# calebki/phylostan

Hardware: AMD Instinct MI355X
Metric: log-lik+grad evals/sec (HKY+W4, 69 taxa) at 1/2/4/8 MI355X; HBM-BW fraction (higher is better)
Workload: dtype f64; 1 GPU; fluA HKY+W4 strict clock, 8192 parameter draws per step; taxa=69, patterns=238, patterns_per_rank=238, categories=4, branches=136, parallelism=replicas1

## Files before the change

### include/phylo_hip_diag.h

```cpp
#ifndef PHYLO_HIP_DIAG_H
#define PHYLO_HIP_DIAG_H

#include "phylo_hip.h"

#ifdef __cplusplus
extern "C" {
#endif

int phy_program_info(const phy_ctx* ctx, int* nsteps, int* nslots, int* depth, int* nblocks);

int phy_plan_records(int S, const int32_t* peel, int rooted, int C, int R, int cols, int cap, int recompute,
                     int32_t* program, int32_t* records, int* nmat, int* n_chunks);

int phy_set_clade_compression(phy_ctx* ctx, int mode);
int phy_clade_compression(const phy_ctx* ctx, int* mode, int* facts, int* clades);

int phy_clade_plan(int S, int P, int C, int rooted, const uint8_t* tipcodes, const int32_t* peel, int R, int cap,
                   int recompute, int mode, int* facts, int* clades, int32_t* program, int32_t* records,
                   int32_t* mat_branch, int32_t* cls_of, int32_t* members, int32_t* rep);

#define PHY_PLAN_QUAD 13
#define PHY_PLAN_CLADE 17
#define PHY_PLAN_LAUNCH 29
#define PHY_PLAN_FACTS 36
int phy_plan_sweep(int S, int P, int C, int rooted, const uint8_t* tipcodes, const int32_t* peel, int max_draws,
                   int cu_count, int wg_budget, int cols, int lds_budget, int deep, int recompute, int clade_mode,
                   int rescaling, int n_draws, int* facts);

int phy_timing_start(phy_ctx* ctx);
int phy_timing_read(phy_ctx* ctx, double* total_ms, int* launches);

int phy_set_tuning(phy_ctx* ctx, int wg_budget, int cols, int lds_budget);

int phy_lds_plan(const phy_ctx* ctx, int* n_chunks, int* matrices_per_chunk, int* lds_bytes);

int phy_columns_per_lane(const phy_ctx* ctx);

int phy_set_deep_stack(phy_ctx* ctx, int mode);
int phy_deep_stack_in_lds(const phy_ctx* ctx);

int phy_set_recompute(phy_ctx* ctx, int on);
int phy_recomputed_partials(const phy_ctx* ctx);

int phy_set_engine(phy_ctx* ctx, int mode);
int phy_engine(const phy_ctx* ctx);

int phy_set_rescaling(phy_ctx* ctx, int on);
int phy_rescaling(const phy_ctx* ctx);

int phy_class_info(const phy_ctx* ctx, long long* classes, int* levels, int* root_classes, long long* stage,
                   long long* staged, int* tiles, int* spans);

int phy_class_clades(const phy_ctx* ctx, int* fused_levels, int* clades, long long* largest);

int phy_class_chain(const phy_ctx* ctx, int* levels, int* lowest, int* top_classes);

int phy_class_fused(const phy_ctx* ctx, int* level_pairs, int* chunk_spans, int* parent_order_levels);

int phy_quad_plan(const phy_ctx* ctx, int* waves, int* span, int* slots);

int phy_geo_info(const phy_geo_ctx* ctx, int* levels, int* widest_level, int* lds_bytes, int* threads,
                 int* workgroups);
int phy_geo_sweeps(phy_geo_ctx* ctx, int n_draws, int* sweeps);
int phy_geo_trees_info(const phy_geo_trees_ctx* ctx, int* widest_level, int* max_levels, int* groups, int* threads,
                       int* lds_bytes, int* workgroups);
int phy_forest_info(const phy_forest_ctx* ctx, int* cols, int* cap_m, int* max_chunks, int* min_chunks,
                    int* max_depth, int* min_depth, int* deep_in_lds, int* lds_bytes);
int phy_forest_plan(int S, int P, int C, int rooted, int model, const uint8_t* tipcodes, const double* weights, int T,
                    const int32_t* peels, int max_rows, int cu_count, int* facts, int* chunks, int* depths);

#ifdef __cplusplus
}
#endif
#endif
```

### phylostan_amd/_lib.py

```python
import ctypes
import importlib.abc
import importlib.machinery
import importlib.util
import os

_HERE = os.path.dirname(os.path.abspath(__file__))
LIB_PATH = os.environ.get("PHYLO_HIP_LIB") or os.path.join(_HERE, "libphylo_hip.so")

PHY_JC69, PHY_HKY, PHY_GTR = 0, 1, 2

_lib = None

_c_double_p = ctypes.POINTER(ctypes.c_double)
_c_int_p = ctypes.POINTER(ctypes.c_int)

SIGNATURES = {
    "phy_create": (ctypes.c_int, [ctypes.c_int, ctypes.c_int, ctypes.c_int, ctypes.c_int, ctypes.c_int,
                                  ctypes.c_void_p, ctypes.c_void_p, ctypes.c_void_p, ctypes.c_int,
                                  ctypes.c_int, ctypes.POINTER(ctypes.c_void_p)]),
    "phy_create_multi": (ctypes.c_int, [ctypes.c_int, ctypes.c_int, ctypes.c_int, ctypes.c_int, ctypes.c_int,
                                        ctypes.c_void_p, ctypes.c_void_p, ctypes.c_void_p, ctypes.c_int,
                                        ctypes.c_int, ctypes.c_void_p, ctypes.POINTER(ctypes.c_void_p)]),
    "phy_destroy": (ctypes.c_int, [ctypes.c_void_p]),
    "phy_last_error": (ctypes.c_char_p, []),
    "phy_num_branches": (ctypes.c_int, [ctypes.c_void_p]),
    "phy_output_len": (ctypes.c_int, [ctypes.c_void_p]),
    "phy_program_info": (ctypes.c_int, [ctypes.c_void_p, _c_int_p, _c_int_p, _c_int_p, _c_int_p]),
    "phy_plan_records": (ctypes.c_int, [ctypes.c_int, ctypes.c_void_p, ctypes.c_int, ctypes.c_int, ctypes.c_int,
                                        ctypes.c_int, ctypes.c_int, ctypes.c_int, ctypes.c_void_p,
                                        ctypes.c_void_p, _c_int_p, _c_int_p]),
    "phy_clade_plan": (ctypes.c_int, [ctypes.c_int] * 4 + [ctypes.c_void_p, ctypes.c_void_p] + [ctypes.c_int] * 4 +
                       [ctypes.c_void_p] * 8),
    "phy_plan_sweep": (ctypes.c_int, [ctypes.c_int] * 4 + [ctypes.c_void_p, ctypes.c_void_p] + [ctypes.c_int] * 10 +
                       [ctypes.c_void_p]),
    "phy_set_clade_compression": (ctypes.c_int, [ctypes.c_void_p, ctypes.c_int]),
    "phy_clade_compression": (ctypes.c_int, [ctypes.c_void_p, _c_int_p, ctypes.c_void_p, ctypes.c_void_p]),
    "phy_eval": (ctypes.c_int, [ctypes.c_void_p, ctypes.c_int, ctypes.c_void_p, ctypes.c_void_p,
                                ctypes.c_void_p, ctypes.c_void_p]),
    "phy_eval_submit": (ctypes.c_int, [ctypes.c_void_p, ctypes.c_int, ctypes.c_void_p, ctypes.c_void_p]),
    "phy_eval_wait": (ctypes.c_int, [ctypes.c_void_p, ctypes.c_void_p]),
    "phy_eval_device": (ctypes.c_int, [ctypes.c_void_p, ctypes.c_int, ctypes.c_void_p, ctypes.c_void_p,
                                       ctypes.c_void_p, ctypes.c_void_p, ctypes.c_void_p]),
    "phy_pruning_loglik": (ctypes.c_double, [ctypes.c_void_p, ctypes.c_void_p, ctypes.c_void_p,
                                             ctypes.c_void_p]),
    "phy_sync": (ctypes.c_int, [ctypes.c_void_p]),
    "phy_timing_start": (ctypes.c_int, [ctypes.c_void_p]),
    "phy_timing_read": (ctypes.c_int, [ctypes.c_void_p, _c_double_p, _c_int_p]),
    "phy_set_tuning": (ctypes.c_int, [ctypes.c_void_p, ctypes.c_int, ctypes.c_int, ctypes.c_int]),
    "phy_lds_plan": (ctypes.c_int, [ctypes.c_void_p, _c_int_p, _c_int_p, _c_int_p]),
    "phy_columns_per_lane": (ctypes.c_int, [ctypes.c_void_p]),
    "phy_set_deep_stack": (ctypes.c_int, [ctypes.c_void_p, ctypes.c_int]),
    "phy_deep_stack_in_lds": (ctypes.c_int, [ctypes.c_void_p]),
    "phy_set_recompute": (ctypes.c_int, [ctypes.c_void_p, ctypes.c_int]),
    "phy_recomputed_partials": (ctypes.c_int, [ctypes.c_void_p]),
    "phy_set_engine": (ctypes.c_int, [ctypes.c_void_p, ctypes.c_int]),
    "phy_set_output": (ctypes.c_int, [ctypes.c_void_p, ctypes.c_int]),
    "phy_engine": (ctypes.c_int, [ctypes.c_void_p]),
    "phy_set_rescaling": (ctypes.c_int, [ctypes.c_void_p, ctypes.c_int]),
    "phy_rescaling": (ctypes.c_int, [ctypes.c_void_p]),
    "phy_class_info": (ctypes.c_int, [ctypes.c_void_p, ctypes.POINTER(ctypes.c_longlong), _c_int_p, _c_int_p,
                                      ctypes.POINTER(ctypes.c_longlong), ctypes.POINTER(ctypes.c_longlong),
                                      _c_int_p, _c_int_p]),
    "phy_class_clades": (ctypes.c_int, [ctypes.c_void_p, _c_int_p, _c_int_p, ctypes.POINTER(ctypes.c_longlong)]),
    "phy_class_chain": (ctypes.c_int, [ctypes.c_void_p, _c_int_p, _c_int_p, _c_int_p]),
    "phy_quad_plan": (ctypes.c_int, [ctypes.c_void_p, _c_int_p, _c_int_p, _c_int_p]),
    "phy_class_fused": (ctypes.c_int, [ctypes.c_void_p, _c_int_p, _c_int_p, _c_int_p]),
    "phy_geo_info": (ctypes.c_int, [ctypes.c_void_p, _c_int_p, _c_int_p, _c_int_p, _c_int_p, _c_int_p]),
    "phy_geo_sweeps": (ctypes.c_int, [ctypes.c_void_p, ctypes.c_int, ctypes.c_void_p]),
    "phy_geo_trees_info": (ctypes.c_int, [ctypes.c_void_p] + [_c_int_p] * 6),
    "phy_forest_info": (ctypes.c_int, [ctypes.c_void_p] + [_c_int_p] * 8),
    "phy_forest_plan": (ctypes.c_int, [ctypes.c_int] * 5 + [ctypes.c_void_p, ctypes.c_void_p, ctypes.c_int,
                                                           ctypes.c_void_p, ctypes.c_int, ctypes.c_int] +
                        [ctypes.c_void_p] * 3),
}


GEO_SIGNATURES = {
    "phy_geo_create": (ctypes.c_int, [ctypes.c_int, ctypes.c_int, ctypes.c_void_p, ctypes.c_void_p, ctypes.c_int,
                                      ctypes.c_int, ctypes.POINTER(ctypes.c_void_p)]),
    "phy_geo_destroy": (ctypes.c_int, [ctypes.c_void_p]),
    "phy_geo_num_branches": (ctypes.c_int, [ctypes.c_void_p]),
    "phy_geo_output_len": (ctypes.c_int, [ctypes.c_void_p]),
    "phy_geo_eval": (ctypes.c_int, [ctypes.c_void_p, ctypes.c_int, ctypes.c_void_p, ctypes.c_void_p,
                                    ctypes.c_void_p]),
    "phy_geo_summary_len": (ctypes.c_int, [ctypes.c_void_p]),
    "phy_geo_eval_summaries": (ctypes.c_int, [ctypes.c_void_p, ctypes.c_int, ctypes.c_void_p, ctypes.c_void_p,
                                              ctypes.c_void_p, ctypes.c_void_p]),
    "phy_geo_trees_create": (ctypes.c_int, [ctypes.c_int, ctypes.c_int, ctypes.c_void_p, ctypes.c_int, ctypes.c_void_p,
                                            ctypes.c_void_p, ctypes.c_void_p, ctypes.c_int, ctypes.c_int,
                                            ctypes.POINTER(ctypes.c_void_p)]),
    "phy_geo_trees_destroy": (ctypes.c_int, [ctypes.c_void_p]),
    "phy_geo_trees_num_trees": (ctypes.c_int, [ctypes.c_void_p]),
    "phy_geo_trees_output_len": (ctypes.c_int, [ctypes.c_void_p]),
    "phy_geo_trees_summary_len": (ctypes.c_int, [ctypes.c_void_p]),
    "phy_geo_trees_eval": (ctypes.c_int, [ctypes.c_void_p, ctypes.c_int, ctypes.c_void_p, ctypes.c_void_p,
                                          ctypes.c_void_p]),
    "phy_geo_trees_eval_summaries": (ctypes.c_int, [ctypes.c_void_p, ctypes.c_int, ctypes.c_void_p, ctypes.c_void_p,
                                                    ctypes.c_void_p, ctypes.c_void_p]),
    "phy_geo_trees_clock_output_len": (ctypes.c_int, [ctypes.c_void_p]),
    "phy_geo_trees_eval_clock": (ctypes.c_int, [ctypes.c_void_p, ctypes.c_int, ctypes.c_void_p, ctypes.c_void_p,
                                                ctypes.c_void_p, ctypes.c_void_p]),
    "phy_geo_trees_eval_clock_summaries": (ctypes.c_int, [ctypes.c_void_p, ctypes.c_int, ctypes.c_void_p,
                                                          ctypes.c_void_p, ctypes.c_void_p, ctypes.c_void_p,
                                                          ctypes.c_void_p]),
}


FOREST_SIGNATURES = {
    "phy_forest_create": (ctypes.c_int, [ctypes.c_int] * 5 + [ctypes.c_void_p, ctypes.c_void_p, ctypes.c_int,
                                                             ctypes.c_void_p, ctypes.c_int, ctypes.c_int,
                                                             ctypes.POINTER(ctypes.c_void_p)]),
    "phy_forest_destroy": (ctypes.c_int, [ctypes.c_void_p]),
    "phy_forest_num_trees": (ctypes.c_int, [ctypes.c_void_p]),
    "phy_forest_num_branches": (ctypes.c_int, [ctypes.c_void_p]),
    "phy_forest_output_len": (ctypes.c_int, [ctypes.c_void_p]),
# ... 76 lines not shown
```

### phylostan_amd/csrc/phylo_hip.hip

```cpp

#include <hip/hip_runtime.h>

#include <cmath>
#include <cstdio>
#include <cstring>
#include <memory>
#include <type_traits>

#include "sweep_plan.h"
#include "forest_plan.h"
#include "geo_plan.h"

namespace {

#ifndef PHY_EPI_U
#define PHY_EPI_U 4
#endif
struct Step {
  int x, y;
  int mxo, myo, mvo;
  int gx, gy, gv;
  int vso;
  uint32_t xso, yso;
  int fl, xd, vd, m0, mn, rd;
// ... 79 lines not shown

template <int CTRL>
__device__ __forceinline__ double dpp_d(double v) {
  const int lo = __builtin_amdgcn_mov_dpp(__double2loint(v), CTRL, 0xF, 0xF, false);
  const int hi = __builtin_amdgcn_mov_dpp(__double2hiint(v), CTRL, 0xF, 0xF, false);
  return __hiloint2double(hi, lo);
}
__device__ __forceinline__ void swap32(double& a, double& b) {
  auto l = __builtin_amdgcn_permlane32_swap(__double2loint(a), __double2loint(b), false, false);
  auto h = __builtin_amdgcn_permlane32_swap(__double2hiint(a), __double2hiint(b), false, false);
  a = __hiloint2double(h[0], l[0]);
  b = __hiloint2double(h[1], l[1]);
}
__device__ __forceinline__ void swap16(double& a, double& b) {
  auto l = __builtin_amdgcn_permlane16_swap(__double2loint(a), __double2loint(b), false, false);
  auto h = __builtin_amdgcn_permlane16_swap(__double2hiint(a), __double2hiint(b), false, false);
  a = __hiloint2double(h[0], l[0]);
  b = __hiloint2double(h[1], l[1]);
}
constexpr int DPP_ROW_ROR8 = 0x128;
constexpr int DPP_ROW_HALF_MIRROR = 0x141;
constexpr int DPP_QUAD_XOR1 = 0xB1;
constexpr int DPP_QUAD_XOR2 = 0x4E;

__device__ __forceinline__ double reduce16(double (&v)[16], int lane) {
#pragma unroll
  for (int k = 0; k < 8; ++k) {
    swap32(v[k], v[k + 8]);
    v[k] += v[k + 8];
  }
#pragma unroll
  for (int k = 0; k < 4; ++k) {
    swap16(v[k], v[k + 4]);
    v[k] += v[k + 4];
  }
  {
    const bool hi = lane & 8;
#pragma unroll
    for (int k = 0; k < 2; ++k) {
      const double send = hi ? v[k] : v[k + 2];
      const double keep = hi ? v[k + 2] : v[k];
      v[k] = keep + dpp_d<DPP_ROW_ROR8>(send);
    }
  }
  {
    const bool hi = lane & 4;
    const double send = hi ? v[0] : v[1];
    const double keep = hi ? v[1] : v[0];
    v[0] = keep + dpp_d<DPP_ROW_HALF_MIRROR>(send);
  }
  double s = v[0];
  s += dpp_d<DPP_QUAD_XOR1>(s);
  s += dpp_d<DPP_QUAD_XOR2>(s);
  return s;
}

__device__ __forceinline__ int reduce16_entry(int lane) {
  return ((lane >> 5) & 1) * 8 + ((lane >> 4) & 1) * 4 + ((lane >> 3) & 1) * 2 + ((lane >> 2) & 1);
}

struct SweepArgs {
  const uint8_t* tips;
  const double* weights;
  const double* pmat;
  const double* model;
  double2* scratch;
  double2* dstk;
  double* gslot;
  double* sslot;
  double* site_ll;
  double* out;
  const int* mat_branch;
  const double* eig;
  double* inner;
  int S, P, Ppad, C, nsteps, nslots, ndeep, ndl, nblk, nmat, R, cap_m;
  int B, outlen, g_direct;
  unsigned long long extra;
  int fin;
  const double* blens;
  double* grows;
  long long grows_stride;
  int qfused, kind;
  int* escr;
  union {
    const int* cc;
    const int* tree_of_row;
  };
  union {
    int cc_ncl;
    int fo_stride;
  };
  int cc_nL, cc_ncol, cc_spos, cc_pre, cc_cnt;
};

__device__ __forceinline__ __amdgpu_buffer_rsrc_t make_rsrc(const void* base, uint32_t bytes) {
  const uint64_t a = reinterpret_cast<uint64_t>(base);
  const uint32_t lo = __builtin_amdgcn_readfirstlane((uint32_t)a);
  const uint32_t hi = __builtin_amdgcn_readfirstlane((uint32_t)(a >> 32));
  const uint32_t n = __builtin_amdgcn_readfirstlane(bytes);
  void* p = reinterpret_cast<void*>(((uint64_t)hi << 32) | lo);
  return __builtin_amdgcn_make_buffer_rsrc(p, (short)0, (int)n, 0x00020000);
}
constexpr int LOAD_NT = 2;
#ifndef PHY_STORE_AUX
#define PHY_STORE_AUX 0
#endif
constexpr int STORE_AUX = PHY_STORE_AUX;
__device__ __forceinline__ V4 ld_v4(__amdgpu_buffer_rsrc_t srd, uint32_t off, uint32_t half) {
  const auto lo = __builtin_amdgcn_raw_buffer_load_b128(srd, off, 0, LOAD_NT);
  const auto hi = __builtin_amdgcn_raw_buffer_load_b128(srd, off, half, LOAD_NT);
  V4 r;
  r.x = __hiloint2double((int)lo[1], (int)lo[0]);
  r.y = __hiloint2double((int)lo[3], (int)lo[2]);
  r.z = __hiloint2double((int)hi[1], (int)hi[0]);
  r.w = __hiloint2double((int)hi[3], (int)hi[2]);
  return r;
}

__device__ __forceinline__ void st_v4(__amdgpu_buffer_rsrc_t srd, uint32_t off, uint32_t half, const V4& v) {
  typedef unsigned u4 __attribute__((ext_vector_type(4)));
  const u4 lo = {(unsigned)__double2loint(v.x), (unsigned)__double2hiint(v.x), (unsigned)__double2loint(v.y),
                 (unsigned)__double2hiint(v.y)};
  const u4 hi = {(unsigned)__double2loint(v.z), (unsigned)__double2hiint(v.z), (unsigned)__double2loint(v.w),
                 (unsigned)__double2hiint(v.w)};
  __builtin_amdgcn_raw_buffer_store_b128(lo, srd, off, 0, STORE_AUX);
  __builtin_amdgcn_raw_buffer_store_b128(hi, srd, off, half, STORE_AUX);
}

__device__ __forceinline__ int v4_exp(const V4& v) {
  const double m = fmax(fmax(v.x, v.y), fmax(v.z, v.w));
  return m > 0.0 ? __builtin_amdgcn_frexp_exp(m) - 1 : 0;
}
__device__ __forceinline__ V4 vldexp(const V4& a, int n) {
  return {ldexp(a.x, n), ldexp(a.y, n), ldexp(a.z, n), ldexp(a.w, n)};
}
__device__ __forceinline__ int ld_exp(__amdgpu_buffer_rsrc_t srd, uint32_t off) {
  return (int)__builtin_amdgcn_raw_buffer_load_b32(srd, off, 0, LOAD_NT);
}
__device__ __forceinline__ void st_exp(__amdgpu_buffer_rsrc_t srd, uint32_t off, int e) {
  __builtin_amdgcn_raw_buffer_store_b32((unsigned)e, srd, off, 0, STORE_AUX);
}

#define WAIT_VMCNT0() __builtin_amdgcn_s_waitcnt(0x0F70)

template <int K>
__device__ __forceinline__ void pvec_k(const double* __restrict__ M, const V4 (&v)[K], V4 (&r)[K]) {
  const double2 a01 = *reinterpret_cast<const double2*>(M + 0), a23 = *reinterpret_cast<const double2*>(M + 2);
  const double2 b01 = *reinterpret_cast<const double2*>(M + 4), b23 = *reinterpret_cast<const double2*>(M + 6);
  const double2 c01 = *reinterpret_cast<const double2*>(M + 8), c23 = *reinterpret_cast<const double2*>(M + 10);
  const double2 d01 = *reinterpret_cast<const double2*>(M + 12), d23 = *reinterpret_cast<const double2*>(M + 14);
#pragma unroll
  for (int k = 0; k < K; ++k) {
    const V4 x = v[k];
    r[k].x = fma(d01.x, x.w, fma(c01.x, x.z, fma(b01.x, x.y, a01.x * x.x)));
    r[k].y = fma(d01.y, x.w, fma(c01.y, x.z, fma(b01.y, x.y, a01.y * x.x)));
    r[k].z = fma(d23.x, x.w, fma(c23.x, x.z, fma(b23.x, x.y, a23.x * x.x)));
    r[k].w = fma(d23.y, x.w, fma(c23.y, x.z, fma(b23.y, x.y, a23.y * x.x)));
  }
}
template <int K>
__device__ __forceinline__ void ptvec_k(const double* __restrict__ M, const V4 (&v)[K], V4 (&r)[K]) {
  const double2 a01 = *reinterpret_cast<const double2*>(M + 0), a23 = *reinterpret_cast<const double2*>(M + 2);
  const double2 b01 = *reinterpret_cast<const double2*>(M + 4), b23 = *reinterpret_cast<const double2*>(M + 6);
  const double2 c01 = *reinterpret_cast<const double2*>(M + 8), c23 = *reinterpret_cast<const double2*>(M + 10);
  const double2 d01 = *reinterpret_cast<const double2*>(M + 12), d23 = *reinterpret_cast<const double2*>(M + 14);
#pragma unroll
  for (int k = 0; k < K; ++k) {
    const V4 x = v[k];
    r[k].x = fma(a23.y, x.w, fma(a23.x, x.z, fma(a01.y, x.y, a01.x * x.x)));
    r[k].y = fma(b23.y, x.w, fma(b23.x, x.z, fma(b01.y, x.y, b01.x * x.x)));
    r[k].z = fma(c23.y, x.w, fma(c23.x, x.z, fma(c01.y, x.y, c01.x * x.x)));
    r[k].w = fma(d23.y, x.w, fma(d23.x, x.z, fma(d01.y, x.y, d01.x * x.x)));
  }
}

// ... 196 lines not shown
        E[2] = dpp_d<0xAA>(Ek);
        E[3] = dpp_d<0xFF>(Ek);
        double T[4];
#pragma unroll
        for (int j = 0; j < 4; ++j) {
          const double g0 = dpp_d<0x00>(g[j]), g1 = dpp_d<0x55>(g[j]), gg2 = dpp_d<0xAA>(g[j]),
                       g3 = dpp_d<0xFF>(g[j]);
          T[j] = fma(sV[12 + k], g3, fma(sV[8 + k], gg2, fma(sV[4 + k], g1, fma(sV[k], g0, 0.0))));
        }
#pragma unroll
        for (int l = 0; l < 4; ++l) {
          double hh = 0.0;
#pragma unroll
          for (int j = 0; j < 4; ++j) hh = fma(T[j], sVi[l * 4 + j], hh);
          const double ri = srinv[k * 4 + l];
          const double phi = ri == 0.0 ? t * Ek : (Ek - E[l]) * ri;
          m[l] = fma(hh, phi, m[l]);
        }
      }
    }
    if (near_any) {
      const RowsG rows{a.grows + (size_t)draw * a.grows_stride};
      double m2[4] = {0.0, 0.0, 0.0, 0.0};
      for (int idx = vt >> 2; idx < C * B; idx += QG_THREADS / 4) {
        const int c = idx / B, b = idx - c * B;
        const double t = mdl[10 + c] * bl[b], Ek = exp(slam[k] * t);
        double g[4];
        rows(idx, k, g);
        double T[4];
#pragma unroll
        for (int j = 0; j < 4; ++j) {
          const double g0 = dpp_d<0x00>(g[j]), g1 = dpp_d<0x55>(g[j]), gg2 = dpp_d<0xAA>(g[j]),
                       g3 = dpp_d<0xFF>(g[j]);
          T[j] = fma(sV[12 + k], g3, fma(sV[8 + k], gg2, fma(sV[4 + k], g1, fma(sV[k], g0, 0.0))));
        }
        const double E[4] = {dpp_d<0x00>(Ek), dpp_d<0x55>(Ek), dpp_d<0xAA>(Ek), dpp_d<0xFF>(Ek)};
#pragma unroll
        for (int l = 0; l < 4; ++l) {
          if (!phi_is_near(slam[k], slam[l])) continue;
          double hh = 0.0;
#pragma unroll
          for (int j = 0; j < 4; ++j) hh = fma(T[j], sVi[l * 4 + j], hh);
          const double d = slam[k] - slam[l];
          m2[l] = fma(hh, phi_near(d, t, Ek, E[l]) - (Ek - E[l]) * srinv[k * 4 + l], m2[l]);
        }
      }
#pragma unroll
      for (int l = 0; l < 4; ++l) m[l] += m2[l];
    }
#pragma unroll
    for (int u = 0; u < 2; ++u) {
      swap32(m[u], m[u + 2]);
      m[u] += m[u + 2];
    }
    swap16(m[0], m[1]);
    m[0] += m[1];
    m[0] += dpp_d<DPP_ROW_ROR8>(m[0]);
    m[0] += dpp_d<0x124>(m[0]);
    if ((lane & 12) == 0) part[vw * 16 + k * 4 + ((lane >> 5) & 1) * 2 + ((lane >> 4) & 1)] = m[0];
  }
  __syncthreads();
  if (tid < 16) {
    double acc = part[tid];
    for (int w = 1; w < QG_THREADS / 64; ++w) acc += part[w * 16 + tid];
    sM[tid] = acc;
  }
  __syncthreads();
  if (tid < 16) sW[tid] = w_entry(sM, sV, sVi, tid);
  __syncthreads();
  if (tid != 0) return;
  double W[16];
  for (int kk = 0; kk < 16; ++kk) W[kk] = sW[kk];
  q_tail(W, e + EIG_Q, e[EIG_S], mdl, out + o, out + o);
}

#ifdef PHY_STEPTIME
#ifndef TT_DRAW0
#define TT_DRAW0 0
#endif
constexpr int TT_DRAWS = 64, TT_EV = 1024;
__device__ unsigned long long g_tt[TT_DRAWS * 16][TT_EV];
#define TT_MARK(i)                                                                   \
  do {                                                                               \
    if (draw >= TT_DRAW0 && draw < TT_DRAW0 + TT_DRAWS && lane == 0)                 \
      g_tt[(draw - TT_DRAW0) * 16 + wv][(i)] = __builtin_amdgcn_s_memtime();         \
  } while (0)
#else
#define TT_MARK(i) do {} while (0)
#endif
template <int MAXT, int K, bool DL, bool RS, bool CC = false, bool FO = false>
__global__ void __launch_bounds__(MAXT) __attribute__((amdgpu_waves_per_eu(MAXT <= 512 ? PHY_WPE2 : 4)))
    sweep_kernel(SweepArgs a, const int* __restrict__ prog) {
  static_assert(!CC || (K == 2 && !RS), "compressed clades: the two-column unscaled sweep only");
  static_assert(!FO || (!CC && !RS), "forest: the unscaled sweep without clades only");
  const int* matbr = a.mat_branch;
  if constexpr (FO) {
    const int t = __builtin_amdgcn_readfirstlane(a.tree_of_row[blockIdx.y]);
    prog += (size_t)t * a.fo_stride;
    matbr += (size_t)t * a.nmat;
  }
  extern __shared__ __attribute__((aligned(16))) unsigned char lds_raw[];
  const int lane = threadIdx.x & (WAVE - 1);
  const int C = a.C, nsteps = a.nsteps, nmat = a.nmat;
  const int wv = __builtin_amdgcn_readfirstlane(threadIdx.x >> 6);
  const int c = wv;
  const int nthreads = blockDim.x;
  const int draw = blockIdx.y;
  const int wg = blockIdx.y * gridDim.x + blockIdx.x;
  const int rec = a.R * 4;
  const int ncolwg = C * WAVE;

  unsigned char* tipl = lds_raw;
  double* tvec = reinterpret_cast<double*>(lds_raw + tip_nib_bytes(a.S, K));
  double* mats0 = tvec + 64;
  if (threadIdx.x < 64) {
    const unsigned b = threadIdx.x >> 2, j = threadIdx.x & 3;
    const unsigned m = b < 4 ? (1u << b) : (unsigned)(a.extra >> (4 * (b - 4))) & 15u;
    tvec[threadIdx.x] = (double)((m >> j) & 1u);
  }
  double* mats = mats0 + (size_t)c * a.cap_m * rec;
  const int ndl = DL ? a.ndeep : a.ndl;
  double* tail0 = mats0 + (size_t)C * a.cap_m * rec;
  const size_t tstride = tail_doubles(K, ndl);

  const double* mdl = a.model + (size_t)draw * (10 + 2 * C);
  const V4 pi = {mdl[0], mdl[1], mdl[2], mdl[3]};
  const double ps_c = mdl[10 + C + c];
  const double* pmat_c = a.pmat + ((size_t)draw * C + c) * nmat * rec;
  const size_t entry2 = (size_t)K * 2 * ncolwg;
  double2* scr = a.scratch + (size_t)wg * a.nslots * entry2;
  double2* dsk = a.dstk + (size_t)wg * a.ndeep * entry2;
  const uint32_t scr_bytes = (uint32_t)((size_t)a.nslots * entry2 * 16);
  const uint32_t dsk_bytes = (uint32_t)((size_t)a.ndeep * entry2 * 16);
  const __amdgpu_buffer_rsrc_t srd_scr = make_rsrc(scr, scr_bytes);
  const __amdgpu_buffer_rsrc_t srd_dsk = make_rsrc(dsk, dsk_bytes);
  const int colw = c * WAVE + lane;
  const uint32_t half_bytes = (uint32_t)ncolwg * 16u;
  const uint32_t estr = (uint32_t)(K * 2 * ncolwg * 16);
  uint32_t lcol[K];
#pragma unroll
  for (int k = 0; k < K; ++k) lcol[k] = (uint32_t)((k * 2 * ncolwg + colw) * 16);
  auto ent = [&](bool use, int e) __attribute__((always_inline)) -> uint32_t {
    return use ? (uint32_t)e * estr : OOB;
  };
  uint32_t lofs[K];
  __amdgpu_buffer_rsrc_t srd_esc = srd_scr;
  uint32_t eofs[K];
  int Eacc[K];
  if constexpr (RS) {
    int* esc = a.escr + (size_t)wg * a.nslots * K * ncolwg;
    srd_esc = make_rsrc(esc, (uint32_t)((size_t)a.nslots * K * ncolwg * 4));
  }
  auto put =[&](double2* base, int e, int k, const V4& v) __attribute__((always_inline)) {
    double2* d = base + ((size_t)e * K + k) * 2 * ncolwg + colw;
    d[0] = make_double2(v.x, v.y);
    d[ncolwg] = make_double2(v.z, v.w);
  };
  double2* dlw = reinterpret_cast<double2*>(tail0 + (size_t)wv * tstride);
  auto dput = [&](int e, int k, const V4& v) __attribute__((always_inline)) {
    double2* d = dlw + (size_t)(e * K + k) * 2 * WAVE + lane;
    d[0] = make_double2(v.x, v.y);
    d[WAVE] = make_double2(v.z, v.w);
  };
  auto dget = [&](int e, int k) __attribute__((always_inline)) -> V4 {
    const double2* d = dlw + (size_t)(e * K + k) * 2 * WAVE + lane;
    const double2 lo = d[0], hi = d[WAVE];
    return V4(lo.x, lo.y, hi.x, hi.y);
  };

  double* gs = a.gslot + ((size_t)wg * C + c) * nmat * 16;
  const int e = reduce16_entry(lane);
  const bool gowner = (lane & 3) == 0;
  char* const gsl = reinterpret_cast<char*>(gs + e);
  bool gstore = gowner, gadd = false;
  auto step_at = [&](int s) __attribute__((always_inline)) -> Step { return ld_step<K>(prog, s, rec * 8, estr); };

  double acc_ll = 0.0, acc_dps = 0.0;
  V4 acc_f = {0.0, 0.0, 0.0, 0.0};

  int cur = -1;
  auto ensure_chunk = [&](const Step& st) {
    const int lo = st.m0, n = st.mn;
    if (lo == cur) return;
    const double2* src = reinterpret_cast<const double2*>(pmat_c + (size_t)lo * rec);
    double2* dst = reinterpret_cast<double2*>(mats);
    const int q2 = n * rec / 2;
    for (int k0 = lane; k0 < q2; k0 += WAVE * 8) {
      double2 buf[8];
#pragma unroll
      for (int u = 0; u < 8; ++u) {
        const int k = k0 + u * WAVE;
        buf[u] = (k < q2) ? src[k] : make_double2(0.0, 0.0);
      }
#pragma unroll
      for (int u = 0; u < 8; ++u) {
        const int k = k0 + u * WAVE;
        if (k < q2) dst[k] = buf[u];
      }
    }
    WAIT_VMCNT0();
    cur = lo;
  };
  const unsigned char* const matb = reinterpret_cast<const unsigned char*>(mats);
  auto mrec = [&](int mo) __attribute__((always_inline)) -> const double* {
    return reinterpret_cast<const double*>(matb + mo);
  };
  const unsigned char* const tipw = tipl + (lane >> 1);
  const unsigned nsh = (lane & 1) * 4;
  auto tipb = [&](int to, int k) __attribute__((always_inline)) -> unsigned {
    return __builtin_amdgcn_ubfe((unsigned)tipw[to + k * (WAVE / 2)], nsh, 4u);
  };
  auto look = [&](int mo, unsigned b) __attribute__((always_inline)) -> V4 {
    const unsigned char* p = matb + mo + (b << 5);
    const double2 lo = *reinterpret_cast<const double2*>(p);
    const double2 hi = *reinterpret_cast<const double2*>(p + 16);
    return {lo.x, lo.y, hi.x, hi.y};
  };
  auto gacc = [&](int go, const V4 (&r)[K], const V4 (&p)[K]) __attribute__((always_inline)) {
    double v[16];
    v[0] = r[0].x * p[0].x;  v[1] = r[0].x * p[0].y;  v[2] = r[0].x * p[0].z;  v[3] = r[0].x * p[0].w;
    v[4] = r[0].y * p[0].x;  v[5] = r[0].y * p[0].y;  v[6] = r[0].y * p[0].z;  v[7] = r[0].y * p[0].w;
    v[8] = r[0].z * p[0].x;  v[9] = r[0].z * p[0].y;  v[10] = r[0].z * p[0].z; v[11] = r[0].z * p[0].w;
    v[12] = r[0].w * p[0].x; v[13] = r[0].w * p[0].y; v[14] = r[0].w * p[0].z; v[15] = r[0].w * p[0].w;
#pragma unroll
    for (int k = 1; k < K; ++k) {
      v[0] = fma(r[k].x, p[k].x, v[0]);   v[1] = fma(r[k].x, p[k].y, v[1]);
      v[2] = fma(r[k].x, p[k].z, v[2]);   v[3] = fma(r[k].x, p[k].w, v[3]);
      v[4] = fma(r[k].y, p[k].x, v[4]);   v[5] = fma(r[k].y, p[k].y, v[5]);
      v[6] = fma(r[k].y, p[k].z, v[6]);   v[7] = fma(r[k].y, p[k].w, v[7]);
      v[8] = fma(r[k].z, p[k].x, v[8]);   v[9] = fma(r[k].z, p[k].y, v[9]);
      v[10] = fma(r[k].z, p[k].z, v[10]); v[11] = fma(r[k].z, p[k].w, v[11]);
      v[12] = fma(r[k].w, p[k].x, v[12]); v[13] = fma(r[k].w, p[k].y, v[13]);
      v[14] = fma(r[k].w, p[k].z, v[14]); v[15] = fma(r[k].w, p[k].w, v[15]);
    }
    const double sum = reduce16(v, lane);
    double* const d = reinterpret_cast<double*>(gsl + (uint32_t)go);
    if (gstore) *d = sum;
    if (gadd) unsafeAtomicAdd(d, sum);
  };

  const int VG = gridDim.x, vg = blockIdx.x;
  const int trips = CC ? a.nblk + 2 : (a.nblk - vg + VG - 1) / VG;
  const uint32_t cw = (uint32_t)c * (WAVE * 16);
  const uint32_t plane_half = (uint32_t)a.nblk * (estr / 2);
  const uint32_t cwp = (uint32_t)c * (uint32_t)a.nblk * (WAVE * K * 16);
  for (int trip = 0; trip < trips; ++trip) {
    const bool passLF = CC && trip == 0, passLR = CC && trip == trips - 1;
    const int blk = CC ? ((passLF || passLR) ? a.nblk : trip - 1) : vg + trip * VG;
    const int f0 = CC ? ((passLF || passLR) ? 0 : a.cc_nL) : 0;
    const int f1 = CC ? (passLF ? a.cc_nL : passLR ? 0 : nsteps) : nsteps;
    const int plim = (CC && (passLF || passLR)) ? a.nblk * (WAVE * K) + a.cc_ncol : a.P;
    TT_MARK(trip * 320 + 0);
#pragma unroll
    for (int k = 0; k < K; ++k) lofs[k] = (blk * WAVE * K + k * WAVE + lane < plim) ? lcol[k] : OOB;
    if constexpr (RS) {
#pragma unroll
      for (int k = 0; k < K; ++k) {
        eofs[k] = (blk * WAVE * K + k * WAVE + lane < a.P) ? (uint32_t)((k * ncolwg + colw) * 4) : OOB;
        Eacc[k] = 0;
      }
    }
    __syncthreads();
    {
      const uint32_t* src = reinterpret_cast<const uint32_t*>(a.tips);
      uint32_t* dst = reinterpret_cast<uint32_t*>(tipl);
      const int rowq = a.Ppad / 8;
      constexpr int wq = WAVE * K / 8;
      const int nq = a.S * wq;
      const int nthr = C * WAVE, t0 = c * WAVE + lane;
      for (int k0 = t0; k0 < nq; k0 += nthr * 8) {
        uint32_t buf[8];
#pragma unroll
        for (int u = 0; u < 8; ++u) {
          const int k = k0 + u * nthr;
          buf[u] = (k < nq) ? src[(size_t)(k / wq) * rowq + blk * wq + (k % wq)] : 0u;
        }
#pragma unroll
        for (int u = 0; u < 8; ++u) {
          const int k = k0 + u * nthr;
          if (k < nq) dst[k] = buf[u];
        }
      }
    }
    __syncthreads();
    WAIT_VMCNT0();
    TT_MARK(trip * 320 + 1);

    V4 top[K], proot[K];
#pragma unroll
    for (int k = 0; k < K; ++k) top[k] = proot[k] = {0.0, 0.0, 0.0, 0.0};
    #define GATHER(ch, so, out) do {                                                         \
      const int* gt_ = a.cc + CC_HDR + ((-2 - (ch)) * a.nblk + blk) * (WAVE * K) + lane;     \
      uint32_t gc_[K];                                                                       \
      _Pragma("unroll")                                                                      \
      for (int k = 0; k < K; ++k) gc_[k] = (uint32_t)gt_[k * WAVE] + cw;                     \
      _Pragma("unroll")                                                                      \
      for (int k = 0; k < K; ++k) out[k] = ld_v4(srd_scr, gc_[k] + (so), half_bytes);        \
      WAIT_VMCNT0();                                                                         \
    } while (0)
    #define FSTEP(s, dcur, dnext, st, sn) do {                                            \
      {                                                                                   \
        const bool more = s + 1 < f1;                                                     \
        sn = step_at(more ? s + 1 : s);                     \
          \
        const bool need = more && (sn.fl & F_XDEEP) && sn.xd >= ndl;                      \
        if (!DL)                                                                                                      \
      _Pragma("unroll")                                                                                               \
        for (int k = 0; k < K; ++k) dnext[k] = ld_v4(srd_scr, lofs[k] + (need ? sn.xso : OOB), half_bytes);    \
      }                                                                                                               \
      ensure_chunk(st);                                                                                               \
      const int x = st.x, y = st.y, fl = st.fl, vso = st.vso;                      \
      V4 ax[K], ay[K], pv[K];                                                                                         \
      if (y >= 0) {                                                                                                   \
        const int my = st.myo;                                                                                    \
      _Pragma("unroll")                                                                                               \
        for (int k = 0; k < K; ++k) ay[k] = look(my, tipb(y, k));                                                     \
      } else if (CC && y < -1) {                                                                                      \
        GATHER(y, st.yso, ay);                                                                                        \
      } else {                                                                                                        \
      _Pragma("unroll")                                                                                               \
        for (int k = 0; k < K; ++k) ay[k] = top[k];                                                                   \
      }                                                                                                               \
      if (x >= 0) {                                                                                                   \
        const int mx = st.mxo;                                                                                    \
      _Pragma("unroll")                                                                                               \
        for (int k = 0; k < K; ++k) ax[k] = look(mx, tipb(x, k));                                                     \
      } else if (CC && x < -1) {                                                                                      \
        GATHER(x, st.xso, ax);                                                                                        \
      } else if (CC ? y != -1 : y >= 0) {                                                                             \
      _Pragma("unroll")                                                                                               \
        for (int k = 0; k < K; ++k) ax[k] = top[k];                                                                   \
      } else {                                                                                                        \
        {                                                                                                             \
          const int xd = st.xd;                                                                                \
          if (DL || xd < ndl) {                                                                                       \
      _Pragma("unroll")                                                                                               \
            for (int k = 0; k < K; ++k) ax[k] = dget(xd, k);                                                          \
          } else {                                                                                                    \
      _Pragma("unroll")                                                                                               \
            for (int k = 0; k < K; ++k) ax[k] = dcur[k];                                                              \
          }                                                                                                           \
        }                                                                                                             \
      }                                                                                                               \
      _Pragma("unroll")                                                                                               \
      for (int k = 0; k < K; ++k) pv[k] = vmul(ax[k], ay[k]);                                                         \
      if (vso >= 0) {                                                                                                 \
        V4 av[K];                                                                                                     \
        if (fl & F_MV) {                                                                                              \
          pvec_k<K>(mrec(st.mvo), pv, av);                                                                        \
        } else {                                                 \
      _Pragma("unroll")                                                                                               \
          for (int k = 0; k < K; ++k) av[k] = pv[k];                                                                  \
        }                                                                                                             \
        if constexpr (RS) {                           \
          if (!(fl & F_NOSTORE)) {                                                                                    \
      _Pragma("unroll")                                                                                               \
            for (int k = 0; k < K; ++k) {                                                                             \
              const int ev = v4_exp(av[k]);                                                                           \
              av[k] = vldexp(av[k], -ev);                                                                             \
              Eacc[k] += ev;                                                                                          \
              st_exp(srd_esc, eofs[k] + ((uint32_t)vso >> 3), ev);                                                    \
            }                                                                                                         \
          }                                                                                                           \
        }                                                                                                             \
      _Pragma("unroll")                                                                                               \
        for (int k = 0; k < K; ++k) if (!(fl & F_NOSTORE)) st_v4(srd_scr, lofs[k] + (uint32_t)vso, half_bytes, av[k]);                                    \
        if (fl & F_VDEEP) {                                                                                           \
          const int dp = st.vd;                                                                                \
          if (DL || dp < ndl)                                          \
          for (int k = 0; k < K; ++k) dput(dp, k, av[k]);                                                             \
        }                                                                                                             \
      _Pragma("unroll")                                                                                               \
        for (int k = 0; k < K; ++k) top[k] = av[k];                                                                   \
      } else {                                                                                                        \
      _Pragma("unroll")                                                                                               \
        for (int k = 0; k < K; ++k) proot[k] = pv[k];                                                                 \
      }                                                                                                               \
    } while (0)
    {
      V4 dA[K], dB[K];
#pragma unroll
// ... 12 lines not shown
    TT_MARK(trip * 320 + 152);

    double fp[K];
    int Est[K], Ed[K];
    if constexpr (RS) {
#pragma unroll
      for (int k = 0; k < K; ++k) {
        fp[k] = vdot(pi, proot[k]);
        *reinterpret_cast<int*>(&tail0[(size_t)wv * tstride + k * WAVE + lane]) = fp[k] > 0.0 ? Eacc[k] : INT_MIN;
      }
      __syncthreads();
#pragma unroll
      for (int k = 0; k < K; ++k) {
        int es = INT_MIN;
        for (int cc = 0; cc < C; ++cc)
          es = max(es, *reinterpret_cast<const int*>(&tail0[(size_t)cc * tstride + k * WAVE + lane]));
        Est[k] = es == INT_MIN ? 0 : es;
      }
      __syncthreads();
#pragma unroll
      for (int k = 0; k < K; ++k) {
        Ed[k] = min(Eacc[k] - Est[k], RS_DMAX);
        fp[k] = ldexp(fp[k], Ed[k]);
        tail0[(size_t)wv * tstride + k * WAVE + lane] = ps_c * fp[k];
      }
    } else {
#pragma unroll
    for (int k = 0; k < K; ++k) {
      fp[k] = vdot(pi, proot[k]);
      tail0[(size_t)wv * tstride + k * WAVE + lane] = ps_c * fp[k];
    }
    }
    __syncthreads();
    double L[K];
#pragma unroll
    for (int k = 0; k < K; ++k) {
      L[k] = 0.0;
      for (int cc = 0; cc < C; ++cc) L[k] += tail0[(size_t)cc * tstride + k * WAVE + lane];
    }
    __syncthreads();
    TT_MARK(trip * 320 + 153);
    V4 topr[K];
#pragma unroll
    for (int k = 0; k < K; ++k) {
      const int i = blk * WAVE * K + k * WAVE + lane;
      const bool live = i < a.P;
      const double wt = a.weights[i];
      double lnL = live ? log(L[k]) : 0.0;
      if constexpr (RS) {
        if (live) lnL = fma((double)Est[k], 0.69314718055994530942, lnL);
      }
      if (c == 0) {
        acc_ll += wt * lnL;
        if (a.site_ll != nullptr && live) a.site_ll[(size_t)draw * a.P + i] = lnL;
      }
      const double sc = live ? wt / L[k] : 0.0;
      double s_c = sc * ps_c;
      if constexpr (RS) s_c = ldexp(s_c, Ed[k]);
      acc_dps = fma(sc, fp[k], acc_dps);
      acc_f.x = fma(s_c, proot[k].x, acc_f.x);
      acc_f.y = fma(s_c, proot[k].y, acc_f.y);
      acc_f.z = fma(s_c, proot[k].z, acc_f.z);
      acc_f.w = fma(s_c, proot[k].w, acc_f.w);
      topr[k] = vscale(pi, s_c);
    }

    struct CSet {
      V4 lx[K], ly[K], lr[K];
      Step st;
      int ex[K], ey[K];
    };
    #define LOAD_SET(s, r) do {                                                  \
      const bool ok = s >= rlo;                                                  \
      r.st = step_at(ok ? s : rlo);                                              \
                                                      \
      const uint32_t xso = ok ? r.st.xso : OOB, yso = ok ? r.st.yso : OOB;       \
      const bool lr = ok && (r.st.fl & F_VDEEP) && r.st.vd >= ndl;               \
      const int vd = r.st.vd;                                                    \
      uint32_t cx_[K], cy_[K];                                                   \
      _Pragma("unroll")                                                          \
      for (int k = 0; k < K; ++k) cx_[k] = cy_[k] = lofs[k];                     \
      if constexpr (CC) {   \
        if (ok && r.st.x < -1) {                                                 \
          const int* gt_ = a.cc + CC_HDR + ((-2 - r.st.x) * a.nblk + blk) * (WAVE * K) + lane;  \
      _Pragma("unroll")                                                          \
          for (int k = 0; k < K; ++k) cx_[k] = (uint32_t)gt_[k * WAVE] + cw;     \
          WAIT_VMCNT0();                                                         \
        }                                                                        \
        if (ok && r.st.y < -1) {                                                 \
          const int* gt_ = a.cc + CC_HDR + ((-2 - r.st.y) * a.nblk + blk) * (WAVE * K) + lane;  \
      _Pragma("unroll")                                                          \
          for (int k = 0; k < K; ++k) cy_[k] = (uint32_t)gt_[k * WAVE] + cw;     \
          WAIT_VMCNT0();                                                         \
        }                                                                        \
      }                                                                          \
      _Pragma("unroll")                                                          \
      for (int k = 0; k < K; ++k) {                                              \
        r.lx[k] = ld_v4(srd_scr, cx_[k] + xso, half_bytes);                      \
        r.ly[k] = ld_v4(srd_scr, cy_[k] + yso, half_bytes);                      \
        if constexpr (!DL)                                                       \
          r.lr[k] = ld_v4(srd_dsk, lcol[k] + ent(lr, vd), half_bytes);            \
        if constexpr (RS) {                                                      \
          r.ex[k] = ld_exp(srd_esc, eofs[k] + (xso >> 3));                       \
          r.ey[k] = ld_exp(srd_esc, eofs[k] + (yso >> 3));                       \
        }                                                                        \
      }                                                                          \
    } while (0)
    #define REBUILD(cst, out) do {   \
      V4 p_[K];                                                                                     \
      _Pragma("unroll")                                                                             \
      for (int k = 0; k < K; ++k)                                                                   \
        p_[k] = vmul(look(cst.mxo, tipb(cst.x, k)), look(cst.myo, tipb(cst.y, k)));                   \
      pvec_k<K>(mrec(cst.mvo), p_, out);                                                            \
    } while (0)
    #define CHAIN_UP(vst, in, out) do {                                                   \
      V4 pu_[K];                                                                          \
      if (vst.x >= 0) {                                                                   \
      _Pragma("unroll")                                                                   \
        for (int k = 0; k < K; ++k) pu_[k] = vmul(look(vst.mxo, tipb(vst.x, k)), in[k]);  \
      } else {                                                                            \
      _Pragma("unroll")                                                                   \
        for (int k = 0; k < K; ++k) pu_[k] = vmul(in[k], look(vst.myo, tipb(vst.y, k))); \
      }                                                                                   \
      pvec_k<K>(mrec(vst.mvo), pu_, out);                                                 \
    } while (0)
    #define REBUILDN(vst, s, d, out) do {                                                 \
      if (d == 1) {                                                                       \
        REBUILD(vst, out);                                                                \
      } else {                                                                            \
        const Step cb_ = step_at(s - d);                                                          \
        V4 acc_[K];                                                                       \
        REBUILD(cb_, acc_);                                                               \
        for (int j_ = d - 1; j_ >= 2; --j_) {                                             \
          const Step v_ = step_at(s - j_);                                                        \
          CHAIN_UP(v_, acc_, acc_);                                                       \
        }                                                                                 \
        CHAIN_UP(vst, acc_, out);                                                         \
      }                                                                                   \
    } while (0)
    #define PLANE_PUT(ch, po, r) do {                                                    \
      const int* sp_ = a.cc + a.cc_spos + ((-2 - (ch)) * a.nblk + blk) * (WAVE * K) + lane;  \
      uint32_t so_[K];                                                                   \
      _Pragma("unroll")                                                                  \
      for (int k = 0; k < K; ++k) so_[k] = (uint32_t)sp_[k * WAVE] + cwp + (uint32_t)(po);  \
      WAIT_VMCNT0();                                                                     \
      _Pragma("unroll")                                                                  \
      for (int k = 0; k < K; ++k) st_v4(srd_scr, so_[k], plane_half, r[k]);              \
    } while (0)
    #define RSTEP_V(s, cs, cn, XT, YT) do {                                               \
      const Step& st = cs.st;                                                     \
      ensure_chunk(st);                                                           \
      const int fl = st.fl;                                                       \
      V4 rv[K], ax[K], ay[K], q[K], rx[K], ry[K];                                 \
      unsigned bx[K], by[K];                                                      \
      if (fl & F_VDEEP) {                                                         \
        const int vd = st.vd;                                                     \
        if (DL || vd < ndl) {                                                     \
      _Pragma("unroll")                                                           \
          for (int k = 0; k < K; ++k) rv[k] = dget(vd, k);                        \
        } else {                                                                  \
      _Pragma("unroll")                                                           \
          for (int k = 0; k < K; ++k) rv[k] = cs.lr[k];                           \
        }                                                                         \
      } else {                                                                    \
      _Pragma("unroll")                                                           \
        for (int k = 0; k < K; ++k) rv[k] = topr[k];                              \
      }                                                                           \
      if (XT) {                                                                   \
        const int mx = st.mxo, x = st.x;                                          \
      _Pragma("unroll")                                                           \
        for (int k = 0; k < K; ++k) {                                             \
          bx[k] = tipb(x, k);                                                     \
          ax[k] = look(mx, bx[k]);                                                \
        }                                                                         \
      } else if (YT && (fl & F_PREVREC)) {   \
        REBUILDN(cn.st, s, st.rd, ax);                                                 \
      } else {                                                                         \
      _Pragma("unroll")                                                                \
        for (int k = 0; k < K; ++k) ax[k] = cs.lx[k];                                  \
      }                                                                           \
      if (YT) {                                                                   \
        const int my = st.myo, y = st.y;                                          \
      _Pragma("unroll")                                                           \
        for (int k = 0; k < K; ++k) {                                             \
          by[k] = tipb(y, k);                                                     \
          ay[k] = look(my, by[k]);                                                \
        }                                                                         \
      } else if (fl & F_PREVREC) {   \
        REBUILDN(cn.st, s, st.rd, ay);                                         \
      } else {                                                                 \
      _Pragma("unroll")                                                        \
        for (int k = 0; k < K; ++k) ay[k] = cs.ly[k];                          \
      }                                                                           \
      if (fl & F_MV) {                                                            \
        V4 pv[K];                                                                 \
      _Pragma("unroll")                                                           \
        for (int k = 0; k < K; ++k) pv[k] = vmul(ax[k], ay[k]);                   \
        ptvec_k<K>(mrec(st.mvo), rv, q);                                          \
        gacc(st.gv, rv, pv);                          \
      } else {                     \
      _Pragma("unroll")                                                           \
        for (int k = 0; k < K; ++k) q[k] = rv[k];                                 \
      }                                                                           \
      _Pragma("unroll")                                                           \
      for (int k = 0; k < K; ++k) {                                               \
        rx[k] = vmul(q[k], ay[k]);                                                \
        ry[k] = vmul(q[k], ax[k]);                                                \
        if constexpr (RS) {     \
          if (!XT) rx[k] = vldexp(rx[k], -cs.ex[k]);                              \
          if (!YT) ry[k] = vldexp(ry[k], -cs.ey[k]);                              \
        }                                                                         \
      }                                                                           \
      if (XT) {                                                                   \
        V4 tv[K];                                                                 \
      _Pragma("unroll")                                                           \
        for (int k = 0; k < K; ++k) tv[k] = tipvec_l(tvec, bx[k]);                \
        gacc(st.gx, rx, tv);                                                      \
      }                                                                           \
      if (YT) {                                                                   \
        V4 tv[K];                                                                 \
      _Pragma("unroll")                                                           \
        for (int k = 0; k < K; ++k) tv[k] = tipvec_l(tvec, by[k]);                \
        gacc(st.gy, ry, tv);                                                      \
      }                                                                           \
                                  \
      if (CC && !XT && st.x < -1) PLANE_PUT(st.x, st.gx, rx);                     \
      if (CC && !YT && st.y < -1) PLANE_PUT(st.y, st.gy, ry);                     \
      if (!XT && !YT) {   \
        if (CC && (st.x < -1 || st.y < -1)) {   \
          if (st.y == -1) {                                                       \
      _Pragma("unroll")                                                           \
            for (int k = 0; k < K; ++k) topr[k] = ry[k];                          \
          } else {                                                                \
      _Pragma("unroll")                                                           \
            for (int k = 0; k < K; ++k) topr[k] = rx[k];                          \
          }                                                                       \
        } else {                                                                  \
        const int dp = st.xd;                                                     \
      _Pragma("unroll")                                                           \
        for (int k = 0; k < K; ++k) {                                             \
          if (DL || dp < ndl) dput(dp, k, rx[k]); else put(dsk, dp, k, rx[k]);    \
          topr[k] = ry[k];                                                        \
        }                                                                         \
        }                                                                         \
      } else if (!YT) {                                                           \
      _Pragma("unroll")                                                           \
        for (int k = 0; k < K; ++k) topr[k] = ry[k];                              \
      } else if (!XT) {                                                           \
      _Pragma("unroll")                                                           \
        for (int k = 0; k < K; ++k) topr[k] = rx[k];                              \
      }                                                                           \
    } while (0)
    #define RSTEP(s, cs, cn) do {                        \
      const int xt_ = cs.st.x >= 0, yt_ = cs.st.y >= 0;  \
      if (xt_ && yt_) RSTEP_V(s, cs, cn, true, true);    \
      else if (xt_) RSTEP_V(s, cs, cn, true, false);     \
      else if (yt_) RSTEP_V(s, cs, cn, false, true);     \
      else RSTEP_V(s, cs, cn, false, false);             \
    } while (0)
    const int nseg = CC ? (passLF ? 0 : passLR ? a.cc_ncl : 1) : 1;
    for (int sg = nseg - 1; sg >= 0; --sg) {
      int rlo = CC ? a.cc_nL : 0, rhi = nsteps - 1;
      if constexpr (CC) {
        if (passLR) {
          rlo = a.cc[4 * sg];
          rhi = a.cc[4 * sg + 1];
          const int mm = a.cc[4 * sg + 3];
          uint32_t pre[K], cnt[K];
#pragma unroll
          for (int k = 0; k < K; ++k) {
            pre[k] = (uint32_t)a.cc[a.cc_pre + sg * (WAVE * K) + k * WAVE + lane] + cwp +
                     (uint32_t)(nsteps + sg * a.nblk) * estr;
            cnt[k] = (uint32_t)a.cc[a.cc_cnt + sg * (WAVE * K) + k * WAVE + lane];
          }
#pragma unroll
          for (int k = 0; k < K; ++k) topr[k] = {0.0, 0.0, 0.0, 0.0};
          for (int t = 0; t < mm; t += CC_ROUNDS_U) {
            V4 rr[CC_ROUNDS_U][K];
#pragma unroll
            for (int u = 0; u < CC_ROUNDS_U; ++u)
#pragma unroll
              for (int k = 0; k < K; ++k)
                rr[u][k] = ld_v4(srd_scr, (uint32_t)(t + u) < cnt[k] ? pre[k] + (uint32_t)(t + u) * 16u : OOB, plane_half);
#pragma unroll
            for (int u = 0; u < CC_ROUNDS_U; ++u)
#pragma unroll
              for (int k = 0; k < K; ++k) {
                topr[k].x += rr[u][k].x;
                topr[k].y += rr[u][k].y;
                topr[k].z += rr[u][k].z;
                topr[k].w += rr[u][k].w;
              }
          }
          WAIT_VMCNT0();
        }
      }
      int s = rhi;
      CSet A, Bs;
      LOAD_SET(s, A);
      for (;;) {
        TT_MARK(trip * 320 + 154 + (nsteps - 1 - s));
        LOAD_SET(s - 1, Bs);
        RSTEP(s, A, Bs);
        if (--s < rlo) break;
        TT_MARK(trip * 320 + 154 + (nsteps - 1 - s));
        LOAD_SET(s - 1, A);
        RSTEP(s, Bs, A);
        if (--s < rlo) break;
      }
    }
    WAIT_VMCNT0();
    TT_MARK(trip * 320 + 310);
    if constexpr (CC) {
      gstore = gowner && (trip == 0 || trip == trips - 2);
      gadd = gowner && !gstore;
    } else {
    gstore = false;
    gadd = gowner;
    }
  }

  acc_ll = wave_sum(acc_ll);
  acc_dps = wave_sum(acc_dps);
  acc_f.x = wave_sum(acc_f.x);
  acc_f.y = wave_sum(acc_f.y);
  acc_f.z = wave_sum(acc_f.z);
  acc_f.w = wave_sum(acc_f.w);
  if (lane == 0) {
    double* ss = a.sslot + ((size_t)wg * C + c) * 8;
    ss[0] = acc_ll;
    ss[1] = acc_dps;
    ss[2] = acc_f.x;
    ss[3] = acc_f.y;
    ss[4] = acc_f.z;
    ss[5] = acc_f.w;
  }
  if (a.g_direct) {
    WAIT_VMCNT0();
    TT_MARK(990);
    double* innerL = mats0;
    double* scalL = mats0 + (size_t)C * a.B;
    if (a.fin) __syncthreads();
    const double* Qd = a.eig + (size_t)draw * EIG_LEN + EIG_Q;
    double* gout = a.grows + (size_t)draw * a.grows_stride;
    double* inner_d = a.inner + (size_t)draw * C * a.B;
    const int e16 = lane & 15, j = e16 >> 2, kk = e16 & 3;
    const double q0 = Qd[j * 4 + 0], q1 = Qd[j * 4 + 1], q2 = Qd[j * 4 + 2], q3 = Qd[j * 4 + 3];
    const int tot = nmat * 16;
    constexpr int U = PHY_EPI_U;
    for (int k0 = lane; k0 < tot; k0 += WAVE * U) {
      double g[U], qp[U];
      int bb[U];
#pragma unroll
      for (int u = 0; u < U; ++u) {
        const int k = k0 + u * WAVE;
        const int kc = k < tot ? k : lane;
// ... 720 lines not shown
    for (int w = 1; w < QFIN_THREADS / 64; ++w) acc += wpart[w][t];
    __hip_atomic_store(hp + t, acc, __ATOMIC_RELAXED, __HIP_MEMORY_SCOPE_AGENT);
  }
  if (tid >= 128 && tid < 128 + C) {
    const int cc = tid - 128;
    double acc = 0.0;
    for (int j = 0; j < nb; ++j) acc = fma(blv[b0 + j], sinner[cc * bper + j], acc);
    __hip_atomic_store(hp + 16 + cc, acc, __ATOMIC_RELAXED, __HIP_MEMORY_SCOPE_AGENT);
  }
  if (sp == 0 && tid == 0) {
    const double ll = sred[0];
    out[0] = isfinite(ll) ? ll : -INFINITY;
    for (int cc = 0; cc < C; ++cc) out[1 + B + C + cc] = sred[cc * 8 + 1];
    for (int f = 0; f < 4; ++f) {
      double t = 0.0;
      for (int cc = 0; cc < C; ++cc) t += sred[cc * 8 + 2 + f];
      __hip_atomic_store(out + o + f, t, __ATOMIC_RELAXED, __HIP_MEMORY_SCOPE_AGENT);
    }
  }
  asm volatile("s_waitcnt vmcnt(0)" ::: "memory");
  __syncthreads();
  if (tid == 0) {
    const unsigned long long old = __hip_atomic_fetch_add(qa.cnt + draw, 1ull, __ATOMIC_RELAXED,
                                                          __HIP_MEMORY_SCOPE_AGENT);
    const bool last = ((old + 1) % (unsigned long long)nspl) == 0;
    handoff_acquire(last);
    s_last = last;
  }
  __syncthreads();
  if (!s_last) return;
  __builtin_amdgcn_fence(__ATOMIC_ACQUIRE, "wavefront");
  const double* pp = qa.part + (size_t)draw * nspl * (16 + C);
  auto ld1 = [](const double* q) { return __hip_atomic_load(q, __ATOMIC_RELAXED, __HIP_MEMORY_SCOPE_AGENT); };
  if (tid < 16) {
    double u[8];
    double acc = 0.0;
    for (int q0 = 0; q0 < nspl; q0 += 8) {
#pragma unroll
      for (int v = 0; v < 8; ++v) u[v] = q0 + v < nspl ? ld1(pp + (size_t)(q0 + v) * (16 + C) + tid) : 0.0;
#pragma unroll
      for (int v = 0; v < 8; ++v)
        if (q0 + v < nspl) acc = (q0 + v == 0) ? u[v] : acc + u[v];
    }
    sM[tid] = acc;
  }
  if (tid >= 64 && tid < 64 + C) {
    const int cc = tid - 64;
    double u[8];
    double acc = 0.0;
    for (int q0 = 0; q0 < nspl; q0 += 8) {
#pragma unroll
      for (int v = 0; v < 8; ++v) u[v] = q0 + v < nspl ? ld1(pp + (size_t)(q0 + v) * (16 + C) + 16 + cc) : 0.0;
#pragma unroll
      for (int v = 0; v < 8; ++v)
        if (q0 + v < nspl) acc = (q0 + v == 0) ? u[v] : acc + u[v];
    }
    out[1 + B + cc] = acc;
  }
  if (!qp) {
    if (tid < 10) out[o + 4 + tid] = 0.0;
    return;
  }
  __syncthreads();
  if (tid < 16) wpart[0][tid] = w_entry(sM, sV, sVi, tid);
  __syncthreads();
  if (tid != 0) return;
  double W[16];
  for (int t = 0; t < 16; ++t) W[t] = wpart[0][t];
  const double rt[4] = {ld1(out + o), ld1(out + o + 1), ld1(out + o + 2), ld1(out + o + 3)};
  q_tail(W, sQ, eg[EIG_S], mdl, rt, out + o);
}

}

namespace {
struct ClassEngine;
void free_class_engine(ClassEngine* e);
struct MultiState;
void free_multi(MultiState* m);

struct CladeBuffers {
  uint8_t* tips = nullptr;
  double* w = nullptr;
  int *prog = nullptr, *tab = nullptr;
  int *matbr = nullptr, *gpos = nullptr;
};
}

struct phy_ctx {
  Problem pb;
  Prefs prefs;
  SweepPlan plan;
  QuadPlan quad;
  CladePlan cc;
  CladeBuffers ccd;
  int device = 0;
  int wg_cap = 0;
  int *d_qprog = nullptr, *d_mprog = nullptr;
  double* d_qscr = nullptr;
  double* d_qfpart = nullptr;
  unsigned long long* d_qfcnt = nullptr;
  long qscr_wgs = 0;
  int* d_escr = nullptr;
  ClassEngine* ce = nullptr;
  MultiState* ms = nullptr;
  int compact = 0;
  double* d_grows = nullptr;
  hipStream_t stream = nullptr;
  hipEvent_t ev_nin = nullptr, ev_nout = nullptr;
  uint8_t* d_tips = nullptr;
  double* d_w = nullptr;
  int *d_prog = nullptr, *d_gpos = nullptr, *d_mat_branch = nullptr;
  double *d_pmat = nullptr, *d_eig = nullptr, *d_inner = nullptr;
  double *d_model = nullptr, *d_blens = nullptr, *d_out = nullptr, *d_site = nullptr;
  double* h_in = nullptr;
  double* h_out = nullptr;
  double* d_in = nullptr;
  int pending = 0;
  double2 *d_scratch = nullptr, *d_dstk = nullptr;
  double *d_gslot = nullptr, *d_sslot = nullptr;
  bool timing = false;
  std::vector<hipEvent_t> ev;
  int ev_used = 0, timed_n = 0;
  double timed_ms = 0.0;
};

namespace {

void free_ctx(phy_ctx* c) {
  if (!c) return;
  int dev_old = 0;
  (void)hipGetDevice(&dev_old);
  (void)hipSetDevice(c->device);
  void* ptrs[] = {c->d_tips,  c->d_w,     c->d_prog,    c->d_gpos,    c->d_mat_branch, c->d_pmat,
                  c->d_eig,   c->d_inner, c->d_model,   c->d_blens,   c->d_out,        c->d_site,
                  c->d_scratch, c->d_dstk, c->d_gslot,  c->d_sslot, c->d_grows, c->d_in, c->d_qprog, c->d_qscr,
                  c->d_qfpart, c->d_qfcnt, c->d_mprog, c->d_escr,
                  c->ccd.tips, c->ccd.w, c->ccd.prog, c->ccd.tab, c->ccd.matbr, c->ccd.gpos};
  for (void* p : ptrs)
    if (p) (void)hipFree(p);
  if (c->h_in) (void)hipHostFree(c->h_in);
  if (c->h_out) (void)hipHostFree(c->h_out);
  for (hipEvent_t e : c->ev) (void)hipEventDestroy(e);
  if (c->ev_nin) (void)hipEventDestroy(c->ev_nin);
  if (c->ev_nout) (void)hipEventDestroy(c->ev_nout);
  free_class_engine(c->ce);
  free_multi(c->ms);
  if (c->stream) (void)hipStreamDestroy(c->stream);
  (void)hipSetDevice(dev_old);
  delete c;
}

template <typename T>
int dalloc(T** p, size_t n) {
  if (n == 0) n = 1;
  hipError_t e = hipMalloc(reinterpret_cast<void**>(p), n * sizeof(T));
  if (e != hipSuccess)
    return fail(PHY_ENOMEM, std::string("hipMalloc ") + std::to_string(n * sizeof(T)) + " B: " +
                                hipGetErrorString(e));
  return PHY_OK;
}

template <typename T, typename U>
int upload(T* dst, const std::vector<U>& src) {
  static_assert(sizeof(T) == sizeof(U), "element sizes differ");
  HIP_TRY(hipMemcpy(dst, src.data(), src.size() * sizeof(U), hipMemcpyHostToDevice));
  return PHY_OK;
}

#include "class_engine.inc"

constexpr int PIN_DRAWS = 128;

struct SweepKernel { int K; bool lat, dl, rs, cc; const void* fn; };
const void* sweep_kernel_cc(bool dl);
const SweepKernel SWEEP_KERNELS[] = {
    {2, false, true, true, false, (const void*)sweep_kernel<512, 2, true, true>},
    {2, false, false, true, false, (const void*)sweep_kernel<512, 2, false, true>},
    {1, true, true, true, false, (const void*)sweep_kernel<512, 1, true, true>},
    {1, true, false, true, false, (const void*)sweep_kernel<512, 1, false, true>},
    {1, false, true, true, false, (const void*)sweep_kernel<1024, 1, true, true>},
    {1, false, false, true, false, (const void*)sweep_kernel<1024, 1, false, true>},
    {2, false, true, false, false, (const void*)sweep_kernel<512, 2, true, false>},
    {2, false, false, false, false, (const void*)sweep_kernel<512, 2, false, false>},
    {1, true, true, false, false, (const void*)sweep_kernel<512, 1, true, false>},
    {1, true, false, false, false, (const void*)sweep_kernel<512, 1, false, false>},
    {1, false, true, false, false, (const void*)sweep_kernel<1024, 1, true, false>},
    {1, false, false, false, false, (const void*)sweep_kernel<1024, 1, false, false>},
    {2, false, true, false, true, sweep_kernel_cc(true)},
    {2, false, false, false, true, sweep_kernel_cc(false)},
};
const void* sweep_kernel_for(int K, bool lat, bool dl, bool rs, bool cc) {
  for (const SweepKernel& k : SWEEP_KERNELS)
    if (k.K == K && k.lat == (lat && K == 1) && k.dl == dl && k.rs == rs && k.cc == cc) return k.fn;
  return nullptr;
}

int alloc_wg_buffers(phy_ctx* c, long cap);

int scratch_slots(const phy_ctx* c) {
  return c->cc.ncl > 0 ? std::max(c->pb.nslots, clade_nslots(c->cc, c->pb.S)) : c->pb.nslots;
}

int build_clade_plan(phy_ctx* c) {
  CladeBuffers& d = c->ccd;
  void* old[] = {d.tips, d.w, d.prog, d.tab, d.matbr, d.gpos};
  for (void* p : old)
    if (p) (void)hipFree(p);
  d = CladeBuffers();
  c->plan.cc_ok = false;
  const Problem& pb = c->pb;
  int rc = select_clades(pb, c->prefs.cc_mode, c->cc);
  if (rc) return rc;
  const CladePlan& cp = c->cc;
  if (cp.ncl == 0) return PHY_OK;
  const std::vector<uint8_t> tips = pack_tips(pb, &cp);
  std::vector<double> w(pb.Ppad + CC_COLS, 0.0);
  std::copy(pb.w.begin(), pb.w.end(), w.begin());
  std::vector<int> gpos(pb.B, -1);
  for (int m = 0; m < cp.nmat; ++m) gpos[cp.mat_branch[m]] = m;
  const std::vector<int> tab = clade_table(cp, pb.S, pb.C);
  if ((rc = dalloc(&d.tips, tips.size())) || (rc = dalloc(&d.w, w.size())) ||
      (rc = dalloc(&d.prog, (size_t)(pb.S - 1) * USTEP)) || (rc = dalloc(&d.tab, tab.size())) ||
      (rc = dalloc(&d.matbr, (size_t)cp.nmat)) || (rc = dalloc(&d.gpos, gpos.size())))
    return rc;
  if ((rc = upload(d.tips, tips)) || (rc = upload(d.w, w)) || (rc = upload(d.tab, tab)) ||
      (rc = upload(d.matbr, cp.mat_branch)))
    return rc;
  return upload(d.gpos, gpos);
}

int upload_clade_records(phy_ctx* c, SweepPlan& plan) {
  std::vector<int> recs;
  int rc = plan_clade_records(c->pb, c->prefs, c->cc, plan, recs);
  if (rc || !plan.cc_ok) return rc;
  return upload(c->ccd.prog, recs);
}

int plan_chunks(phy_ctx* c) {
  SweepPlan plan = c->plan;
  int rc = plan_lds(c->pb, c->prefs, plan.cu_count, plan);
  if (rc) return rc;
  if (plan.wg_need > c->wg_cap) {
    HIP_TRY(hipStreamSynchronize(c->stream));
    if ((rc = alloc_wg_buffers(c, plan.wg_need))) return rc;
    c->wg_cap = (int)plan.wg_need;
  }
  if ((rc = upload(c->d_prog, plan.records))) return rc;
  if ((rc = upload_clade_records(c, plan))) return rc;
  c->plan = std::move(plan);
  return PHY_OK;
}

int select_engine(phy_ctx* c) {
  const Problem& pb = c->pb;
  c->plan.engine = 0;
  if (c->prefs.rescale) return PHY_OK;
  if (c->prefs.engine == 1 || (c->prefs.engine == 0 && pb.P < 16384)) return PHY_OK;
  int rc = c->ce ? PHY_OK
                 : build_class_engine(pb.S, pb.P, pb.C, pb.rooted, pb.tips.data(), pb.w.data(), pb.peel.data(),
                                      pb.vec_of, pb.R, pb.nmat, pb.gpos, &c->ce);
  if (rc) return rc;
  const double pattern_work = (double)(pb.S - 2) * pb.P;
  if (c->prefs.engine == 2 || (double)c->ce->classes <= 0.25 * pattern_work) {
    c->plan.engine = 1;
  } else {
    free_class_engine(c->ce);
    c->ce = nullptr;
  }
  return PHY_OK;
}

int timing_fold(phy_ctx* ctx) {
  for (int k = 0; k + 1 < ctx->ev_used; k += 2) {
    HIP_TRY(hipEventSynchronize(ctx->ev[k + 1]));
    float ms = 0.f;
    HIP_TRY(hipEventElapsedTime(&ms, ctx->ev[k], ctx->ev[k + 1]));
    ctx->timed_ms += ms;
    ctx->timed_n += 1;
  }
  ctx->ev_used = 0;
  return PHY_OK;
}

int timing_begin(phy_ctx* ctx, hipStream_t st, hipEvent_t* e0, hipEvent_t* e1) {
  if (ctx->ev_used + 2 > (int)ctx->ev.size()) {
    int rc = timing_fold(ctx);
    if (rc) return rc;
  }
  *e0 = ctx->ev[ctx->ev_used];
  *e1 = ctx->ev[ctx->ev_used + 1];
  ctx->ev_used += 2;
  HIP_TRY(hipEventRecord(*e0, st));
  return PHY_OK;
}

int output_len(const phy_ctx* ctx) {
  return PHY_OUT_G(ctx->pb.B, ctx->pb.C) + (ctx->compact ? 0 : 16 * ctx->pb.C * ctx->pb.B);
}

struct CallBufs {
  const double *blens, *model;
  double *out, *site;
  double* grows;
  long long gstride;
};

SweepArgs sweep_args(const phy_ctx* ctx, const LaunchChoice& ch, const CallBufs& io) {
  const Problem& pb = ctx->pb;
  const SweepPlan& pl = ctx->plan;
  SweepArgs a{};
  a.tips = ctx->d_tips; a.weights = ctx->d_w; a.pmat = ctx->d_pmat; a.mat_branch = ch.mat_branch; a.eig = ch.eig;
  a.model = io.model; a.blens = io.blens; a.site_ll = io.site; a.out = io.out;
  a.grows = io.grows; a.grows_stride = io.gstride; a.outlen = output_len(ctx);
  a.scratch = ctx->d_scratch; a.dstk = ctx->d_dstk; a.gslot = ctx->d_gslot; a.sslot = ctx->d_sslot;
  a.inner = ctx->d_inner; a.escr = ctx->prefs.rescale ? ctx->d_escr : nullptr;
  a.S = pb.S; a.P = pb.P; a.Ppad = pb.Ppad; a.C = pb.C; a.B = pb.B; a.R = pb.R; a.extra = pb.extra; a.kind = pb.kind;
  a.nsteps = pb.nsteps; a.nslots = pb.nslots; a.ndeep = pb.ndeep; a.nmat = pb.nmat; a.nblk = pl.nblk;
  a.ndl = ch.quad() ? 0 : pl.ndl; a.cap_m = ch.quad() ? pb.nmat : pl.cap_m;
  a.g_direct = ch.g_direct; a.fin = ch.fin; a.qfused = ch.qf;
  if (ch.cc()) {
    const CladePlan& cp = ctx->cc;
    a.tips = ctx->ccd.tips; a.weights = ctx->ccd.w; a.Ppad = pb.Ppad + CC_COLS; a.nslots = clade_nslots(cp, pb.S);
    a.cc = ctx->ccd.tab; a.cc_ncl = cp.ncl; a.cc_nL = cp.nL; a.cc_ncol = cp.maxcls;
    a.cc_spos = CC_HDR + cp.ncl * cp.nblk * CC_COLS;
    a.cc_pre = a.cc_spos + cp.ncl * cp.nblk * CC_COLS;
    a.cc_cnt = a.cc_pre + cp.ncl * CC_COLS;
  }
  return a;
}

FinArgs fin_args(const phy_ctx* ctx, const LaunchChoice& ch, const CallBufs& io) {
  const Problem& pb = ctx->pb;
  FinArgs f{};
  f.gslot = ctx->d_gslot; f.sslot = ctx->d_sslot; f.pmat = ctx->d_pmat; f.inner = ctx->d_inner;
  f.eig = ch.eig; f.gpos = ch.gpos; f.blens = io.blens; f.model = io.model; f.out = io.out;
  f.grows = io.grows; f.grows_stride = io.gstride; f.outlen = output_len(ctx);
  f.C = pb.C; f.B = pb.B; f.nmat = pb.nmat; f.R = pb.R; f.kind = pb.kind;
  f.gx = ch.gx; f.g_direct = ch.g_direct; f.gsum_in = ch.gsum_in; f.qf = ch.fin_qf;
  return f;
}

int launch_class(phy_ctx* ctx, const LaunchChoice& ch, int n, const CallBufs& io, hipStream_t st) {
  ClassEngine* e = ctx->ce;
  const int C = ctx->pb.C, B = ctx->pb.B;
  if ((long)n * C > 65535) return fail(PHY_ERANGE, "class sweep: n_draws * C must be <= 65535");
  int rc = class_engine_reserve(e, n, st);
  if (rc) return rc;
  ClassArgs a = class_args(e, ctx->d_pmat, io.model, ctx->pb.extra);
  const int dcn = n * C;
  hipEvent_t e0 = nullptr, e1 = nullptr;
  if (ctx->timing && (rc = timing_begin(ctx, st, &e0, &e1))) return rc;
  if (e->Lc > 0)
    hipLaunchKernelGGL(cls_clade_fwd_kernel, dim3(e->nclade, dcn), dim3(CLADE_THREADS), 0, st, a,
                       (const CladeLevel*)e->d_clade, e->Lc);
  const bool chain = e->chain_m > 0;
  const ChainArgs ca{e->d_link, e->d_ctab, e->d_crep, e->chain_m, e->chain_ntop, e->chain_ntp, e->chain_toff};
  const int chain_wgs = (e->chain_ntp / WAVE + CLS_WPG - 1) / CLS_WPG;
  auto in_chain = [&](int l) { return chain && l >= e->chain_lo && l <= e->chain_hi; };
  for (int l = e->Lc + 1; l < e->levels; ++l) {
    const ClassLevel& L = e->lv[l];
    if (!L.nchunk || in_chain(l) || L.pair == 2) continue;
    a.first = L.chunk0;
    a.count = L.nchunk;
    if (L.pair == 1) {
      a.count += e->lv[l + 1].nchunk;
      hipLaunchKernelGGL(cls_fwd2_kernel, dim3((a.count + CLS_WPG - 1) / CLS_WPG, dcn), dim3(CLS_THREADS), 0, st, a,
                         (const int2*)e->d_pair, (const int4*)e->d_gc);
      continue;
    }
    hipLaunchKernelGGL(cls_fwd_kernel, dim3((L.nchunk + CLS_WPG - 1) / CLS_WPG, dcn), dim3(CLS_THREADS), 0, st, a);
  }
  const bool root_chain = chain && C <= 4 && e->root_chain_pref;
  if (chain && !root_chain)
    hipLaunchKernelGGL(e->chain_m <= 4 ? cls_chain_fwd_kernel<4> : e->chain_m == 5 ? cls_chain_fwd_kernel<5>
                       : e->chain_m <= 6 ? cls_chain_fwd_kernel<6> : cls_chain_fwd_kernel<CHAIN_MAX>,
                       dim3(chain_wgs, dcn), dim3(CLS_THREADS), 0, st, a, ca);
  auto rk = C <= 4 ? (e->root_tips ? cls_root_kernel<256, true> : cls_root_kernel<256, false>)
                   : (e->root_tips ? cls_root_kernel<1024, true> : cls_root_kernel<1024, false>);
  if (root_chain) {
    const int m = e->chain_m;
    rk = e->root_tips ? (m <= 4 ? cls_root_kernel<256, true, 4> : m == 5 ? cls_root_kernel<256, true, 5>
                         : m <= 6 ? cls_root_kernel<256, true, 6> : cls_root_kernel<256, true, CHAIN_MAX>)
                      : (m <= 4 ? cls_root_kernel<256, false, 4> : m == 5 ? cls_root_kernel<256, false, 5>
                         : m <= 6 ? cls_root_kernel<256, false, 6> : cls_root_kernel<256, false, CHAIN_MAX>);
  }
  hipLaunchKernelGGL(rk, dim3(e->nrootch, n), dim3(C * WAVE), 0, st, a, ca);
  for (int l = e->levels - 1; l > e->Lc; --l) {
    const ClassLevel& L = e->lv[l];
    if (L.ntile) {
      a.first = L.tile0;
      a.count = L.ntile;
      a.sfirst = L.sec0;
      a.sord = L.sord;
      hipLaunchKernelGGL(cls_red_kernel, dim3((L.ntile + CLS_WPG - 1) / CLS_WPG, dcn), dim3(CLS_THREADS), 0, st, a);
    }
    if (L.nlfix && !L.revfix)
      hipLaunchKernelGGL(cls_fix_list_kernel, dim3((L.nlfix + CLS_WPG - 1) / CLS_WPG, dcn), dim3(CLS_THREADS), 0, st, a,
                         (const int*)e->d_lfix + L.lfix0, L.nlfix);
    if (in_chain(l)) {
      if (l == e->chain_hi)
        hipLaunchKernelGGL(e->chain_m <= 4 ? cls_chain_rev_kernel<4> : e->chain_m == 5 ? cls_chain_rev_kernel<5>
                           : e->chain_m <= 6 ? cls_chain_rev_kernel<6> : cls_chain_rev_kernel<CHAIN_MAX>,
                           dim3(chain_wgs, dcn), dim3(CLS_THREADS), 0, st, a, ca);
      continue;
    }
    if (L.nchunk) {
      a.first = L.chunk0;
      a.count = L.nchunk;
      if (L.revfix)
// ... 82 lines not shown
    hipLaunchKernelGGL(qgrad_kernel, dim3(n), dim3(QG_THREADS), 0, st, fin_args(ctx, ch, io));
    HIP_TRY(hipGetLastError());
  }
  return PHY_OK;
}

int launch_quad(phy_ctx* ctx, const LaunchChoice& ch, int n, const CallBufs& io, hipStream_t st) {
  const Problem& pb = ctx->pb;
  const int C = pb.C, gx = ch.gx;
  const long wgs = (long)gx * n;
  int rc = PHY_OK;
  if (wgs > ctx->wg_cap || wgs > ctx->qscr_wgs) {
    HIP_TRY(hipDeviceSynchronize());
    if (wgs > ctx->wg_cap) {
      if ((rc = alloc_wg_buffers(ctx, wgs))) return rc;
      ctx->wg_cap = (int)wgs;
    }
    if (wgs > ctx->qscr_wgs) {
      if (ctx->d_qscr) (void)hipFree(ctx->d_qscr);
      ctx->d_qscr = nullptr;
      ctx->qscr_wgs = 0;
      if ((rc = dalloc(&ctx->d_qscr, (size_t)wgs * std::max(pb.nslots, 1) * C * WAVE))) return rc;
      ctx->qscr_wgs = wgs;
    }
  }
  const int bper = qfin_bper(pb), nspl = qfin_nspl(pb);
  if (!ctx->d_qfcnt) {
    HIP_TRY(hipDeviceSynchronize());
    rc = dalloc(&ctx->d_qfpart, (size_t)QUAD_MAX_DRAWS * nspl * (16 + C));
    if (!rc) rc = dalloc(&ctx->d_qfcnt, (size_t)QUAD_MAX_DRAWS);
    if (rc) return rc;
    HIP_TRY(hipMemset(ctx->d_qfcnt, 0, (size_t)QUAD_MAX_DRAWS * sizeof(unsigned long long)));
    HIP_TRY(hipDeviceSynchronize());
  }
  QuadArgs qa;
  qa.s = sweep_args(ctx, ch, io);
  qa.qscr = ctx->d_qscr;
  qa.nblk = (pb.P + QCOLS - 1) / QCOLS;
  qa.pmat_out = ctx->d_pmat;
  qa.build = ch.quad_build ? 1 : 0;
  hipEvent_t e0 = nullptr, e1 = nullptr;
  if (ctx->timing && (rc = timing_begin(ctx, st, &e0, &e1))) return rc;
  if (ch.path == PATH_QUAD_MW) {
    const QmwPlan& mp = ctx->quad.mw;
    QmwArgs ma{qa, ctx->d_mprog, mp.W, mp.maxst, mp.nslot, mp.root_wave, mp.nst[0], mp.nst[1], mp.nst[2], mp.nst[3]};
    void* kargs[] = {(void*)&ma};
    HIP_TRY(hipLaunchKernel((const void*)qmw_kernel, dim3(gx, n), dim3(C * mp.W * WAVE), kargs, ctx->quad.mw_lds, st));
  } else {
    const int* prog = ctx->d_qprog;
    void* kargs[] = {(void*)&qa, (void*)&prog};
    const void* kern = C <= 4 ? (const void*)qsweep_kernel<256> : (const void*)qsweep_kernel<1024>;
    HIP_TRY(hipLaunchKernel(kern, dim3(gx, n), dim3(C * WAVE), kargs, ctx->quad.lds, st));
  }
  HIP_TRY(hipGetLastError());
  if (ctx->timing) HIP_TRY(hipEventRecord(e1, st));
  const FinArgs fa = fin_args(ctx, ch, io);
  if (ch.qfin) {
    hipLaunchKernelGGL(qfin_kernel, dim3(nspl, n), dim3(QFIN_THREADS), 0, st,
                       QfinArgs{fa, ctx->d_qfpart, ctx->d_qfcnt, bper, nspl});
    HIP_TRY(hipGetLastError());
    return PHY_OK;
  }
  return launch_finalize(ch, fa, n, st);
}

const void* sweep_kernel_cc(bool dl) {
  return dl ? (const void*)sweep_kernel<512, 2, true, false, true> : (const void*)sweep_kernel<512, 2, false, false, true>;
}

int launch_pattern(phy_ctx* ctx, const LaunchChoice& ch, int n, const CallBufs& io, hipStream_t st) {
  const Problem& pb = ctx->pb;
  const SweepPlan& pl = ctx->plan;
  const int C = pb.C, gx = ch.gx;
  int rc = PHY_OK;
  if ((size_t)gx * n > (size_t)ctx->wg_cap) return fail(PHY_ERANGE, "workgroup cap exceeded");
  if (ctx->prefs.rescale && !ctx->d_escr) return fail(PHY_EINVAL, "internal: rescaling without its exponent plane");
  const SweepArgs sa = sweep_args(ctx, ch, io);
  hipEvent_t e0 = nullptr, e1 = nullptr;
  if (ctx->timing && (rc = timing_begin(ctx, st, &e0, &e1))) return rc;
  {
    const int* prog = ch.cc() ? ctx->ccd.prog : ctx->d_prog;
    void* kargs[] = {(void*)&sa, (void*)&prog};
    HIP_TRY(hipLaunchKernel(sweep_kernel_for(pl.K, pl.lat, pl.deep_lds, ctx->prefs.rescale, ch.cc()), dim3(gx, n),
                            dim3(C * WAVE), kargs, pl.lds, st));
  }
  HIP_TRY(hipGetLastError());
  if (ctx->timing) HIP_TRY(hipEventRecord(e1, st));
  return launch_finalize(ch, fin_args(ctx, ch, io), n, st);
}

int alloc_wg_buffers(phy_ctx* c, long cap) {
  const Problem& pb = c->pb;
  const size_t ncolwg = (size_t)pb.C * WAVE;
  double2 *scr = nullptr, *dsk = nullptr;
  double *gsl = nullptr, *ssl = nullptr;
  int* esc = nullptr;
  int rc = dalloc(&scr, (size_t)cap * std::max(scratch_slots(c), 1) * 2 * 2 * ncolwg);
  if (!rc) rc = dalloc(&dsk, (size_t)cap * std::max(pb.ndeep, 1) * 2 * 2 * ncolwg);
  if (!rc) rc = dalloc(&gsl, (size_t)cap * pb.C * pb.nmat * 16);
  if (!rc) rc = dalloc(&ssl, (size_t)cap * pb.C * 8);
  if (!rc && c->prefs.rescale) rc = dalloc(&esc, (size_t)cap * std::max(pb.nslots, 1) * 2 * ncolwg);
  if (rc) {
    const std::string msg = g_err;
    void* ps[] = {scr, dsk, gsl, ssl, esc};
    for (void* p : ps)
      if (p) (void)hipFree(p);
    return fail(rc, msg);
  }
  void* old[] = {c->d_scratch, c->d_dstk, c->d_gslot, c->d_sslot, c->d_escr};
  for (void* p : old)
    if (p) (void)hipFree(p);
  c->d_scratch = scr; c->d_dstk = dsk; c->d_gslot = gsl; c->d_sslot = ssl; c->d_escr = esc;
  return PHY_OK;
}

constexpr int EIG_HOST_MAX = 32;
int eval_small(phy_ctx* ctx, int n, const double* blens, const double* model, double* dsite) {
  const int ml = 10 + 2 * ctx->pb.C;
  const size_t nb = (size_t)n * ctx->pb.B, nm = (size_t)n * ml;
  std::memcpy(ctx->h_in, blens, sizeof(double) * nb);
  std::memcpy(ctx->h_in + nb, model, sizeof(double) * nm);
  const bool host_eig = n <= EIG_HOST_MAX;
  if (host_eig) {
    double* eg = ctx->h_in + nb + nm;
    for (int d = 0; d < n; ++d) eig_record(model + (size_t)d * ml, ctx->pb.kind, eg + (size_t)d * EIG_LEN);
  }
  const size_t nin = nb + nm + (host_eig ? (size_t)n * EIG_LEN : 0);
  hipStream_t st = ctx->stream;
  HIP_TRY(hipMemcpyAsync(ctx->d_in, ctx->h_in, sizeof(double) * nin, hipMemcpyHostToDevice, st));
  const double* in = ctx->d_in;
  int rc = launch(ctx, n, in, in + nb, ctx->d_out, dsite, st, host_eig ? in + nb + nm : nullptr);
  if (rc) return rc;
  HIP_TRY(hipMemcpyAsync(ctx->h_out, ctx->d_out, sizeof(double) * n * output_len(ctx), hipMemcpyDeviceToHost, st));
  return PHY_OK;
}

void quad_facts(const QuadPlan& q, const SweepPlan& plan, const Prefs& prefs, int nsteps, int* waves, int* span,
                int* slots) {
  const bool on = plan.qmw_ok && prefs.qmw;
  if (waves) *waves = on ? q.mw.W : (plan.quad_ok ? 1 : 0);
  if (span) *span = on ? q.mw.span : nsteps;
  if (slots) *slots = on ? q.mw.nslot : 0;
}

}

template <typename F>
int null_fenced(phy_ctx* ctx, F&& body) {
  HIP_TRY(hipEventRecord(ctx->ev_nin, nullptr));
  HIP_TRY(hipStreamWaitEvent(ctx->stream, ctx->ev_nin, 0));
  const int rc = body(ctx->stream);
  if (rc) return rc;
  HIP_TRY(hipEventRecord(ctx->ev_nout, ctx->stream));
  HIP_TRY(hipStreamWaitEvent(nullptr, ctx->ev_nout, 0));
  return PHY_OK;
}

#include "multi_device.inc"

namespace {
phy_ctx* answering(phy_ctx* ctx) { return ctx->ms ? ctx->ms->shard[0] : ctx; }
const phy_ctx* answering(const phy_ctx* ctx) { return answering(const_cast<phy_ctx*>(ctx)); }
template <typename F>
int each_shard(phy_ctx* ctx, F&& set) {
  for (phy_ctx* s : ctx->ms->shard) {
    int rc = set(s);
    if (rc) return rc;
// ... 183 lines not shown
int phy_output_len(const phy_ctx* ctx) { return ctx ? output_len(answering(ctx)) : -1; }

int phy_set_output(phy_ctx* ctx, int compact) {
  if (!ctx) return fail(PHY_EINVAL, "NULL ctx");
  if (ctx->pending || (ctx->ms && ctx->ms->pending))
    return fail(PHY_EINVAL, "phy_set_output: a phy_eval_submit is still in flight (phy_eval_wait first)");
  if (ctx->ms) {
    int rc = each_shard(ctx, [&](phy_ctx* s) { return phy_set_output(s, compact); });
    if (rc) return rc;
    ctx->compact = compact ? 1 : 0;
    return PHY_OK;
  }
  HIP_TRY(hipSetDevice(ctx->device));
  HIP_TRY(hipStreamSynchronize(ctx->stream));
  if (compact && !ctx->d_grows) {
    int rc = dalloc(&ctx->d_grows, (size_t)ctx->pb.max_draws * 16 * ctx->pb.C * ctx->pb.B);
    if (rc) return rc;
  }
  ctx->compact = compact ? 1 : 0;
  return PHY_OK;
}

int phy_plan_records(int S, const int32_t* peel, int rooted, int C, int R, int cols, int cap, int recompute,
                     int32_t* program, int32_t* records, int* nmat, int* n_chunks) {
  if (S < 2 || !peel || C < 1 || R < 4 || (cols != 1 && cols != 2) || cap < 3)
    return fail(PHY_EINVAL, "phy_plan_records: bad argument");
  std::vector<int> prog, mat_branch;
  int nslots = 0, ndeep = 0, nch = 0, nrec = 0;
  int rc = build_program(S, peel, rooted, prog, mat_branch, nslots, ndeep);
  if (rc) return rc;
  rc = assign_chunks(prog, S - 1, (int)mat_branch.size(), cap, recompute != 0, nch, nrec);
  if (rc) return rc;
  const std::vector<int> recs = batched_records(prog, cols, C, R);
  if (program) std::copy(prog.begin(), prog.end(), program);
  if (records) std::copy(recs.begin(), recs.end(), records);
  if (nmat) *nmat = (int)mat_branch.size();
  if (n_chunks) *n_chunks = nch;
  return PHY_OK;
}

int phy_clade_plan(int S, int P, int C, int rooted, const uint8_t* tipcodes, const int32_t* peel, int R, int cap,
                   int recompute, int mode, int* facts, int* clades, int32_t* program, int32_t* records,
                   int32_t* mat_branch, int32_t* cls_of, int32_t* members, int32_t* rep) {
  if (S < 3 || P < 1 || !tipcodes || !peel || C < 1 || C > 8 || R < 4 || cap < 3 || !facts)
    return fail(PHY_EINVAL, "phy_clade_plan: bad argument");
  PeelTree t;
  int rc = parse_peel(S, peel, rooted, t);
  if (rc) return rc;
  CladePlan cp;
  if (mode != 0 && (rc = plan_clades(t, P, tipcodes, mode, cp))) return rc;
  std::vector<int> raw, recs;
  int nch = 0, nrec = 0;
  if (cp.ncl > 0 && (rc = clade_records(cp, S, C, R, cap, recompute != 0, raw, recs, nch, nrec))) return rc;
  clade_facts(cp, S, nch, nrec, cp.ncl > 0, facts, clades);
  if (cp.ncl == 0) return PHY_OK;
  if (program) std::copy(raw.begin(), raw.end(), program);
  if (records) std::copy(recs.begin(), recs.end(), records);
  if (mat_branch) std::copy(cp.mat_branch.begin(), cp.mat_branch.end(), mat_branch);
  if (cls_of) std::copy(cp.cls_of.begin(), cp.cls_of.end(), cls_of);
  if (members) std::copy(cp.members.begin(), cp.members.end(), members);
  if (rep) std::copy(cp.rep.begin(), cp.rep.end(), rep);
  return PHY_OK;
}

int phy_plan_sweep(int S, int P, int C, int rooted, const uint8_t* tipcodes, const int32_t* peel, int max_draws,
                   int cu_count, int wg_budget, int cols, int lds_budget, int deep, int recompute, int clade_mode,
                   int rescaling, int n_draws, int* facts) {
  if (!facts || cu_count < 1 || cols < 0 || cols > 2 || deep < 0 || deep > 2 || clade_mode < -1 || clade_mode > 1)
    return fail(PHY_EINVAL, "phy_plan_sweep: bad argument");
  const std::vector<double> w((size_t)std::max(P, 1), 1.0);
  Problem pb;
  int rc = make_problem(S, P, C, rooted, PHY_JC69, tipcodes, w.data(), peel, max_draws, pb);
  if (rc) return rc;
  if (n_draws < 1 || n_draws > max_draws) return fail(PHY_ERANGE, "n_draws out of range");
  Prefs prefs = prefs_from_env();
  if (wg_budget > 0) prefs.wg_budget = wg_budget;
  if (lds_budget > 0) prefs.lds_budget = std::max(16384, std::min(lds_budget, (int)LDS_CAP));
  prefs.cols = cols; prefs.deep = deep; prefs.recompute = recompute != 0; prefs.cc_mode = clade_mode;
  prefs.rescale = rescaling != 0;
  SweepPlan plan;
  if ((rc = plan_lds(pb, prefs, cu_count, plan))) return rc;
  CladePlan cp;
  std::vector<int> recs;
  if ((rc = select_clades(pb, prefs.cc_mode, cp)) || (rc = plan_clade_records(pb, prefs, cp, plan, recs))) return rc;
  const QuadPlan quad = plan_quad(pb, plan);
  const LaunchChoice ch = choose_launch(pb, prefs, plan, n_draws, n_draws <= EIG_HOST_MAX);
  const int head[PHY_PLAN_QUAD] = {pb.nsteps, pb.nslots, pb.ndeep, pb.R, plan.K, plan.lat ? 1 : 0, plan.nblk,
                                   plan.cap_m, plan.nchunks, plan.ndl, plan.nrec, plan.wg_resident, (int)plan.lds};
  std::copy(head, head + PHY_PLAN_QUAD, facts);
  facts[PHY_PLAN_QUAD] = plan.quad_ok ? 1 : 0;
  quad_facts(quad, plan, prefs, pb.nsteps, facts + PHY_PLAN_QUAD + 1, facts + PHY_PLAN_QUAD + 2, facts + PHY_PLAN_QUAD + 3);
  clade_facts(cp, S, plan.cc_nchunks, plan.cc_nrec, plan.cc_ok && prefs.cc_mode != 0, facts + PHY_PLAN_CLADE, nullptr);
  const int tail[PHY_PLAN_FACTS - PHY_PLAN_LAUNCH] = {ch.path, ch.gx, ch.g_direct, ch.fin, ch.qf, ch.gsum_in,
                                                      ch.quad_build ? 1 : 0};
  std::copy(tail, tail + PHY_PLAN_FACTS - PHY_PLAN_LAUNCH, facts + PHY_PLAN_LAUNCH);
  return PHY_OK;
}

int phy_set_clade_compression(phy_ctx* ctx, int mode) {
  if (!ctx) return fail(PHY_EINVAL, "NULL ctx");
  if (mode < -1 || mode > 1) return fail(PHY_EINVAL, "clade compression mode must be 0 (off), 1 (on) or -1 (automatic)");
  if (ctx->ms) return each_shard(ctx, [&](phy_ctx* s) { return phy_set_clade_compression(s, mode); });
  if (ctx->pending) return fail(PHY_EINVAL, "phy_set_clade_compression: a phy_eval_submit is still in flight");
  if (mode == ctx->prefs.cc_mode) return PHY_OK;
  HIP_TRY(hipSetDevice(ctx->device));
  HIP_TRY(hipStreamSynchronize(ctx->stream));
  const int had = scratch_slots(ctx);
  ctx->prefs.cc_mode = mode;
  int rc = build_clade_plan(ctx);
  if (rc) return rc;
  if (scratch_slots(ctx) > had && (rc = alloc_wg_buffers(ctx, ctx->wg_cap))) {
    ctx->cc = CladePlan();
    ctx->plan.cc_ok = false;
    return rc;
  }
  return upload_clade_records(ctx, ctx->plan);
}

int phy_clade_compression(const phy_ctx* ctx, int* mode, int* facts, int* clades) {
  if (!ctx) return fail(PHY_EINVAL, "NULL ctx");
  ctx = answering(ctx);
  if (mode) *mode = ctx->prefs.cc_mode;
  clade_facts(ctx->cc, ctx->pb.S, ctx->plan.cc_nchunks, ctx->plan.cc_nrec, ctx->plan.cc_ok && ctx->prefs.cc_mode != 0,
              facts, clades);
  return PHY_OK;
}

int phy_program_info(const phy_ctx* ctx, int* nsteps, int* nslots, int* depth, int* nblocks) {
  if (!ctx) return fail(PHY_EINVAL, "NULL ctx");
  ctx = answering(ctx);
  if (nsteps) *nsteps = ctx->pb.nsteps;
  if (nslots) *nslots = ctx->pb.nslots;
  if (depth) *depth = ctx->pb.ndeep;
  if (nblocks) *nblocks = ctx->plan.nblk;
  return PHY_OK;
}

int phy_eval_device(phy_ctx* ctx, int n_draws, const double* d_blens, const double* d_model,
                    double* d_out, double* d_site_ll, void* stream) {
  if (!ctx) return fail(PHY_EINVAL, "NULL ctx");
  if (ctx->ms) return multi_eval_device(ctx, n_draws, d_blens, d_model, d_out, d_site_ll, stream);
  if (n_draws < 1 || n_draws > ctx->pb.max_draws) return fail(PHY_ERANGE, "n_draws out of range");
  if (!d_blens || !d_model || !d_out) return fail(PHY_EINVAL, "NULL device buffer");
  if (ctx->pending)
    return fail(PHY_EINVAL, "phy_eval_device: a phy_eval_submit is still in flight (phy_eval_wait first)");
  HIP_TRY(hipSetDevice(ctx->device));
  if (stream) return launch(ctx, n_draws, d_blens, d_model, d_out, d_site_ll, reinterpret_cast<hipStream_t>(stream));
  return null_fenced(ctx, [&](hipStream_t st) { return launch(ctx, n_draws, d_blens, d_model, d_out, d_site_ll, st); });
}

int phy_eval_submit(phy_ctx* ctx, int n_draws, const double* blens, const double* model) {
  if (!ctx) return fail(PHY_EINVAL, "NULL ctx");
  if (ctx->ms) {
    if (ctx->ms->pending) return fail(PHY_EINVAL, "phy_eval_submit: an evaluation is already in flight");
    if (n_draws < 1 || n_draws > ctx->pb.max_draws || n_draws > PIN_DRAWS)
      return fail(PHY_ERANGE, "phy_eval_submit: n_draws must be in [1, min(max_draws, 128)]");
    if (!blens || !model) return fail(PHY_EINVAL, "NULL host buffer");
    int rc = multi_enqueue(ctx, n_draws, blens, model, false);
    if (rc) return rc;
    ctx->ms->pending = n_draws;
    return PHY_OK;
  }
  if (ctx->pending) return fail(PHY_EINVAL, "phy_eval_submit: an evaluation is already in flight");
  if (n_draws < 1 || n_draws > ctx->pb.max_draws || n_draws > PIN_DRAWS || !ctx->h_in || !ctx->h_out || !ctx->d_in)
    return fail(PHY_ERANGE, "phy_eval_submit: n_draws must be in [1, min(max_draws, 128)]");
  if (!blens || !model) return fail(PHY_EINVAL, "NULL host buffer");
  HIP_TRY(hipSetDevice(ctx->device));
  int rc = eval_small(ctx, n_draws, blens, model, nullptr);
  if (rc) return rc;
  ctx->pending = n_draws;
  return PHY_OK;
}

int phy_eval_wait(phy_ctx* ctx, double* out) {
  if (!ctx) return fail(PHY_EINVAL, "NULL ctx");
  if (ctx->ms) {
    if (!ctx->ms->pending) return fail(PHY_EINVAL, "phy_eval_wait: nothing submitted");
    if (!out) return fail(PHY_EINVAL, "NULL host buffer");
// ... 232 lines not shown
```

### phylostan_amd/csrc/sweep_plan.h

```cpp
#ifndef PHYLO_SWEEP_PLAN_H
#define PHYLO_SWEEP_PLAN_H

#include <algorithm>
#include <climits>
#include <cstdint>
#include <cstdlib>
#include <string>
#include <utility>
#include <vector>

#include "phylo_hip_diag.h"

#if defined(__HIPCC__)
#define PHY_HD __host__ __device__
#else
#define PHY_HD
#endif

namespace {

constexpr int WAVE = 64;
constexpr int STEP_INTS = 16;
enum {
  ST_X = 0,
  ST_Y,
  ST_MX,
  ST_MY,
  ST_MV,
  ST_VSLOT,
  ST_FLAGS,
  ST_XSLOT,
  ST_YSLOT,
  ST_XDPOS,
  ST_VDPOS,
  ST_CHUNK,
  ST_M0,
  ST_MN,
  ST_NODE,
  ST_RD,
};
constexpr int F_MV = 1;
constexpr int F_XDEEP = 2;
constexpr int F_VDEEP = 4;
constexpr int F_NOSTORE = 8;
constexpr int F_PREVREC = 16;
#ifndef PHY_RD_MAX
#define PHY_RD_MAX 4
#endif
constexpr int RD_MAX = PHY_RD_MAX;
constexpr int RS_DMAX = 900;
constexpr int CC_MAXCL = 8;
constexpr int CC_COLS = 128;
constexpr int CC_MININT = 3;
constexpr int CC_ROUNDS_U = 8;
constexpr int CC_HDR = 4 * CC_MAXCL;

constexpr int PSTEP = 8;
enum {
  BR_X = 0,
  BR_Y,
  BR_MXO,
  BR_MYO,
  BR_MVO,
  BR_VSO,
  BR_FLRD,
  BR_XSO,
  BR_YSO,
  BR_XDPOS,
  BR_VDPOS,
  BR_GX,
  BR_M0,
  BR_MN,
  BR_GY,
  BR_GV,
};
constexpr int USTEP = STEP_INTS;
constexpr uint32_t OOB = 0x40000000u;
constexpr int EIG_LEN = 56;
constexpr int EIG_M1 = 0, EIG_LAM = 16, EIG_M2 = 20, EIG_Q = 36, EIG_S = 52;

constexpr int QG_THREADS = 1024;
constexpr int QG_SHARED = 16 * 3 + 4 + (QG_THREADS / 64) * 16 + 16 * 2;
constexpr int QFIN_THREADS = 256;
constexpr int QFIN_ITEMS = QFIN_THREADS / 4;
constexpr int QFIN_SLOTS = 16;

constexpr size_t LDS_CAP = 160 * 1024;
constexpr int MIN_CAP = 24;
#ifndef PHY_WPE2
#define PHY_WPE2 2
#endif

thread_local std::string g_err;

int fail(int code, const std::string& msg) {
  g_err = msg;
  return code;
}

PHY_HD inline size_t tip_nib_bytes(int S, int K) { return ((size_t)S * WAVE * K / 2 + 15) / 16 * 16; }
PHY_HD inline size_t tip_lds_bytes(int S, int K) { return tip_nib_bytes(S, K) + 16 * 4 * sizeof(double); }
PHY_HD inline size_t tail_doubles(int K, int ndl) {
  return ndl > 0 ? (size_t)ndl * K * 2 * WAVE * 2 : (size_t)K * WAVE;
}
PHY_HD inline size_t lds_bytes(int S, int C, int R, int cap_m, int K, int ndl) {
  return tip_nib_bytes(S, K) + 16 * 4 * sizeof(double) + (size_t)C * cap_m * R * 32 +
         (size_t)C * tail_doubles(K, ndl) * 8;
}

inline int nblk_for(int P, int K) { return (P + WAVE * K - 1) / (WAVE * K); }
inline int waves_per_simd(int K, bool lat) { return (K == 2 || lat) ? PHY_WPE2 : 4; }

std::vector<int> pack_program(const std::vector<int>& prog) {
  const size_t n = prog.size() / STEP_INTS;
  std::vector<int> out(n * PSTEP, 0);
  auto h = [](int lo, int hi) { return (int)(((unsigned)(lo & 0xFFFF)) | ((unsigned)hi << 16)); };
  for (size_t s = 0; s < n; ++s) {
    const int* p = &prog[s * STEP_INTS];
    int* q = &out[s * PSTEP];
    q[0] = h(p[ST_X], p[ST_Y]);
    q[1] = h(p[ST_MX], p[ST_MY]);
    q[2] = h(p[ST_MV], p[ST_VSLOT]);
    q[3] = h(p[ST_XSLOT], p[ST_YSLOT]);
    q[4] = (int)((unsigned)(p[ST_FLAGS] & 0xFF) | ((unsigned)(p[ST_XDPOS] & 0xFF) << 8) |
                 ((unsigned)(p[ST_VDPOS] & 0xFF) << 16));
    q[5] = h(p[ST_CHUNK], p[ST_M0]);
    q[6] = h(p[ST_MN], p[ST_NODE]);
    q[7] = p[ST_RD];
  }
  return out;
}

std::vector<int> batched_records(const std::vector<int>& prog, int K, int C, int R, int plane0 = -1, int nblk = 0) {
  const size_t n = prog.size() / STEP_INTS;
  std::vector<int> out(n * USTEP, 0);
  const uint32_t estr = (uint32_t)(K * 2 * C * WAVE * 16);
  const int rec8 = R * 32;
  for (size_t s = 0; s < n; ++s) {
// ... 196 lines not shown
  if ((int)(prog.size() / STEP_INTS) != S - 1) return fail(PHY_EINVAL, "tree is not binary / connected");
  nslots = S - 2;
  return PHY_OK;
}

int assign_chunks(std::vector<int>& prog, int nsteps, int nmat, int cap, bool recompute, int& nchunks, int& nrec,
                  int brk = -1) {
  int used = 0, ch = 0, lo = 0;
  std::vector<int> first_step{0};
  for (int s = 0; s < nsteps; ++s) {
    const int* p = &prog[(size_t)s * STEP_INTS];
    const int n = (p[ST_MX] >= 0) + (p[ST_MY] >= 0) + (p[ST_MV] >= 0);
    if (used + n > cap || (s == brk && s > 0)) {
      first_step.push_back(s);
      lo += used;
      used = 0;
      ++ch;
    }
    int* q = &prog[(size_t)s * STEP_INTS];
    q[ST_CHUNK] = ch;
    q[ST_M0] = lo;
    used += n;
  }
  if (lo + used != nmat) return fail(PHY_EINVAL, "internal: chunk plan does not cover the matrices");
  first_step.push_back(nsteps);
  for (int k = 0; k <= ch; ++k) {
    const int m0 = prog[(size_t)first_step[k] * STEP_INTS + ST_M0];
    const int m1 = (k < ch) ? prog[(size_t)first_step[k + 1] * STEP_INTS + ST_M0] : nmat;
    for (int s = first_step[k]; s < first_step[k + 1]; ++s) prog[(size_t)s * STEP_INTS + ST_MN] = m1 - m0;
  }
  nrec = 0;
  for (int s = 0; s < nsteps; ++s) {
    prog[(size_t)s * STEP_INTS + ST_FLAGS] &= ~(F_NOSTORE | F_PREVREC);
    prog[(size_t)s * STEP_INTS + ST_RD] = 0;
  }
  if (recompute) {
    for (int s = 1; s < nsteps; ++s) {
      int* p = &prog[(size_t)s * STEP_INTS];
      int* q = &prog[(size_t)(s - 1) * STEP_INTS];
      const bool has_internal = p[ST_X] < 0 || p[ST_Y] < 0;
      const bool eligible = (q[ST_FLAGS] & F_MV) && q[ST_VSLOT] >= 0 && !(q[ST_FLAGS] & F_VDEEP);
      if (!has_internal || !eligible || p[ST_X] <= -2 || p[ST_Y] <= -2) continue;
      int d = 0;
      if (q[ST_X] >= 0 && q[ST_Y] >= 0) d = 1;
      else if ((q[ST_X] >= 0) != (q[ST_Y] >= 0) && q[ST_RD] > 0) d = q[ST_RD] + 1;
      if (d == 0 || d > RD_MAX || s - d < 0) continue;
      bool same = true;
      for (int j = 1; j <= d; ++j) same = same && prog[(size_t)(s - j) * STEP_INTS + ST_CHUNK] == p[ST_CHUNK];
      if (!same) continue;
      q[ST_FLAGS] |= F_NOSTORE;
      p[ST_FLAGS] |= F_PREVREC;
      p[ST_RD] = d;
      ++nrec;
    }
  }
  nchunks = ch + 1;
  return PHY_OK;
}

struct CladePlan {
  int ncl = 0;
  int node[CC_MAXCL] = {}, ncls[CC_MAXCL] = {}, maxmult[CC_MAXCL] = {}, nint[CC_MAXCL] = {};
  int lo[CC_MAXCL] = {}, hi[CC_MAXCL] = {};
  int nblk = 0;
  int nL = 0, nU = 0, nmat = 0, nmatL = 0, ndeep = 0, maxcls = 0;
  int rounds = 0;
  std::vector<int> prog;
  std::vector<int> mat_branch;
  std::vector<int> cls_of;
  std::vector<int> members;
  std::vector<int> rep;
  std::vector<char> in_clade;
  std::vector<int> clade_of_tip;
};

constexpr size_t CC_MAX_CELLS = (size_t)1 << 22;

constexpr long CC_STEP_CYCLES = 4700;
constexpr long CC_BOUNDARY_CYCLES = 13000;
constexpr long CC_BATCH_CYCLES = 2500;
constexpr long CC_CLADE_CYCLES = 7000;
constexpr long CC_FIXED_CYCLES = 6000;

int plan_clades(const PeelTree& t, int P, const uint8_t* tipcodes, int mode, CladePlan& cp) {
  const int S = t.S, N = 2 * S - 1;
  cp = CladePlan();
  cp.nblk = (P + CC_COLS - 1) / CC_COLS;
  if (cp.nblk < 2 || (size_t)N * P > CC_MAX_CELLS) return PHY_OK;
  std::vector<int> order;
  {
    std::vector<std::pair<int, int>> st{{t.root, 0}};
    while (!st.empty()) {
      auto& [n, k] = st.back();
      if (n < S) {
        st.pop_back();
        continue;
      }
      if (k == 2) {
        order.push_back(n);
        st.pop_back();
        continue;
      }
      const int child = (k == 0) ? t.ch1[n] : t.ch2[n];
      ++k;
      st.push_back({child, 0});
    }
  }
  std::vector<std::vector<int>> cid(N);
  std::vector<int> count(N, 0), nint(N, 0);
  auto col = [&](int n, int p) -> long { return n < S ? (long)tipcodes[(size_t)n * P + p] : (long)cid[n][p]; };
  for (int v : order) {
    const int a = t.ch1[v], b = t.ch2[v];
    nint[v] = 1 + nint[a] + nint[b];
    if ((a >= S && count[a] < 0) || (b >= S && count[b] < 0)) {
      count[v] = -1;
      continue;
    }
    std::vector<std::pair<long, int>> keys(P);
    for (int p = 0; p < P; ++p) keys[p] = {col(a, p) * 65536 + col(b, p), p};
    std::vector<std::pair<long, int>> sorted = keys;
    std::sort(sorted.begin(), sorted.end());
    std::vector<int> firstp;
    for (int i = 0; i < P; ++i)
      if (i == 0 || sorted[i].first != sorted[i - 1].first) firstp.push_back(sorted[i].second);
    if ((int)firstp.size() > CC_COLS) {
      count[v] = -1;
      continue;
    }
    std::sort(firstp.begin(), firstp.end());
    std::vector<int> idof(P, -1);
    for (int j = 0; j < (int)firstp.size(); ++j) idof[firstp[j]] = j;
    cid[v].assign(P, -1);
    int run = -1;
    for (int i = 0; i < P; ++i) {
      if (i == 0 || sorted[i].first != sorted[i - 1].first) run = idof[sorted[i].second];
      cid[v][sorted[i].second] = run;
    }
    count[v] = (int)firstp.size();
  }
  auto mult_of = [&](int v) {
    std::vector<int> sz(count[v], 0);
    for (int p = 0; p < P; ++p) ++sz[cid[v][p]];
    return *std::max_element(sz.begin(), sz.end());
  };
  long gain = 0;
  std::vector<int> walk{t.root};
  while (!walk.empty()) {
    const int v = walk.back();
    walk.pop_back();
    if (v < S) continue;
    bool take = v != t.root && count[v] > 0 && nint[v] >= CC_MININT && cp.ncl < CC_MAXCL;
    int mm = 0;
    if (take) {
      mm = mult_of(v);
      const long save = (long)(cp.nblk - 1) * nint[v] * CC_STEP_CYCLES;
      const long cost = (long)cp.nblk * CC_BOUNDARY_CYCLES +
                        (long)((mm + CC_ROUNDS_U - 1) / CC_ROUNDS_U) * CC_BATCH_CYCLES + CC_CLADE_CYCLES;
      if (mode != 1 && 4 * save <= 5 * cost) take = false;
      if (take) gain += save - cost;
    }
    if (!take) {
      walk.push_back(t.ch2[v]);
      walk.push_back(t.ch1[v]);
      continue;
    }
    const int ci = cp.ncl++;
    cp.node[ci] = v;
    cp.ncls[ci] = count[v];
    cp.maxmult[ci] = mm;
    cp.nint[ci] = nint[v];
  }
  if (cp.ncl > 0 && mode != 1 && gain <= CC_FIXED_CYCLES) cp.ncl = 0;
  if (cp.ncl == 0) return PHY_OK;
  int mmx = 0;
  for (int ci = 0; ci < cp.ncl; ++ci) {
    mmx = std::max(mmx, cp.maxmult[ci]);
    cp.maxcls = std::max(cp.maxcls, cp.ncls[ci]);
  }
  cp.rounds = (mmx + CC_ROUNDS_U - 1) / CC_ROUNDS_U * CC_ROUNDS_U;
  const int pcols = cp.nblk * CC_COLS;
  cp.cls_of.assign((size_t)cp.ncl * pcols, -1);
  cp.members.assign((size_t)cp.ncl * cp.rounds * CC_COLS, -1);
  cp.rep.assign((size_t)cp.ncl * CC_COLS, -1);
  cp.in_clade.assign(N, 0);
  cp.clade_of_tip.assign(S, -1);
  std::vector<int> gath(N, -1);
  for (int ci = 0; ci < cp.ncl; ++ci) {
    const int v = cp.node[ci];
    gath[v] = ci;
    std::vector<int> fill(CC_COLS, 0);
    for (int p = 0; p < P; ++p) {
      const int j = cid[v][p];
      cp.cls_of[(size_t)ci * pcols + p] = j;
      if (fill[j] == 0) cp.rep[(size_t)ci * CC_COLS + j] = p;
      cp.members[((size_t)ci * cp.rounds + fill[j]++) * CC_COLS + j] = p;
    }
    std::vector<int> st{v};
    while (!st.empty()) {
      const int n = st.back();
      st.pop_back();
      cp.in_clade[n] = 1;
      if (n < S) {
        cp.clade_of_tip[n] = ci;
        continue;
      }
      st.push_back(t.ch1[n]);
      st.push_back(t.ch2[n]);
    }
  }
  std::vector<int> slot(N, -1);
  const std::vector<int> none(N, -1);
  for (int ci = 0; ci < cp.ncl; ++ci) {
    cp.lo[ci] = (int)(cp.prog.size() / STEP_INTS);
    int rc = emit_steps(t, cp.node[ci], none, cp.prog, cp.mat_branch, slot, cp.ndeep);
    if (rc) return rc;
    cp.hi[ci] = (int)(cp.prog.size() / STEP_INTS) - 1;
  }
  cp.nL = (int)(cp.prog.size() / STEP_INTS);
  cp.nmatL = (int)cp.mat_branch.size();
  int rc = emit_steps(t, t.root, gath, cp.prog, cp.mat_branch, slot, cp.ndeep);
  if (rc) return rc;
  cp.nU = (int)(cp.prog.size() / STEP_INTS) - cp.nL;
  cp.nmat = (int)cp.mat_branch.size();
  if (cp.nL + cp.nU != S - 1) return fail(PHY_EINVAL, "internal: L and U do not cover the tree");
  return PHY_OK;
}

int clade_records(const CladePlan& cp, int S, int C, int R, int cap, bool recompute, std::vector<int>& raw,
                  std::vector<int>& recs, int& nchunks, int& nrec) {
  raw = cp.prog;
  int rc = assign_chunks(raw, S - 1, cp.nmat, cap, recompute, nchunks, nrec, cp.nL);
  if (rc) return rc;
  recs = batched_records(raw, 2, C, R, S - 1, cp.nblk);
  return PHY_OK;
}
inline int clade_nslots(const CladePlan& cp, int S) { return S - 1 + cp.ncl * cp.nblk; }

std::vector<int> clade_table(const CladePlan& cp, int S, int C) {
  const int ncolwg = C * WAVE;
  auto colpart = [&](int q) { return (uint32_t)(((q / WAVE) * 2 * ncolwg + (q % WAVE)) * 16); };
  const int pcols = cp.nblk * CC_COLS;
  const size_t o_cls = CC_HDR, o_spos = o_cls + (size_t)cp.ncl * pcols, o_pre = o_spos + (size_t)cp.ncl * pcols,
               o_cnt = o_pre + (size_t)cp.ncl * CC_COLS;
  std::vector<int> tab(o_cnt + (size_t)cp.ncl * CC_COLS, (int)OOB);
  for (int ci = 0; ci < cp.ncl; ++ci) {
    tab[4 * ci] = cp.lo[ci];
    tab[4 * ci + 1] = cp.hi[ci];
    tab[4 * ci + 2] = cp.ncls[ci];
    tab[4 * ci + 3] = cp.maxmult[ci];
    for (int p = 0; p < pcols; ++p) {
      const int j = cp.cls_of[(size_t)ci * pcols + p];
      if (j >= 0) tab[o_cls + (size_t)ci * pcols + p] = (int)colpart(j);
    }
    int run = 0;
    for (int j = 0; j < CC_COLS; ++j) {
      int n = 0;
      for (int r = 0; r < cp.rounds; ++r) {
        const int p = cp.members[((size_t)ci * cp.rounds + r) * CC_COLS + j];
        if (p < 0) break;
        tab[o_spos + (size_t)ci * pcols + p] = (run + n) * 16;
        ++n;
      }
      tab[o_pre + (size_t)ci * CC_COLS + j] = run * 16;
      tab[o_cnt + (size_t)ci * CC_COLS + j] = n;
      run += n;
    }
  }
  (void)S;
  return tab;
}

void clade_facts(const CladePlan& cp, int S, int nchunks, int nrec, bool on, int* facts, int* clades) {
  if (facts) {
    const int fv[12] = {cp.ncl, cp.nL, cp.nU, cp.nmatL, cp.nmat - cp.nmatL, cp.rounds, cp.maxcls, cp.nblk,
                        cp.ncl ? clade_nslots(cp, S) : 0, cp.ndeep, nchunks, nrec};
    for (int k = 0; k < 12; ++k) facts[k] = on ? fv[k] : 0;
  }
  if (clades)
    for (int ci = 0; ci < CC_MAXCL; ++ci) {
      const bool have = on && ci < cp.ncl;
      const int cv[6] = {cp.node[ci], cp.nint[ci], cp.ncls[ci], cp.maxmult[ci], cp.lo[ci], cp.hi[ci]};
      for (int k = 0; k < 6; ++k) clades[6 * ci + k] = have ? cv[k] : 0;
    }
}

constexpr int QCOLS = 16;
constexpr int QUAD_MAX_DRAWS = 32;

enum {
  QS_XT = 0,
  QS_YT,
  QS_MXB,
  QS_MYB,
  QS_MVB,
  QS_VSO,
  QS_FL,
  QS_XSO,
  QS_YSO,
  QS_XDO,
  QS_VDO,
  QS_MXG,
  QS_MYG,
  QS_MVG,
};

std::vector<int> quad_program(const std::vector<int>& prog, int nsteps, int C, int R) {
  std::vector<int> q((size_t)nsteps * STEP_INTS, 0);
  const int recb = R * 4 * 8;
  for (int s = 0; s < nsteps; ++s) {
    const int* p = &prog[(size_t)s * STEP_INTS];
    int* o = &q[(size_t)s * STEP_INTS];
    o[QS_XT] = p[ST_X] >= 0 ? p[ST_X] * (QCOLS / 2) : -1;
    o[QS_YT] = p[ST_Y] >= 0 ? p[ST_Y] * (QCOLS / 2) : -1;
    o[QS_MXB] = p[ST_MX] >= 0 ? p[ST_MX] * recb : 0;
    o[QS_MYB] = p[ST_MY] >= 0 ? p[ST_MY] * recb : 0;
    o[QS_MVB] = p[ST_MV] >= 0 ? p[ST_MV] * recb : 0;
    o[QS_VSO] = p[ST_VSLOT] >= 0 ? p[ST_VSLOT] * C * WAVE : -1;
    o[QS_FL] = p[ST_FLAGS] & ~(F_NOSTORE | F_PREVREC);
    o[QS_XSO] = p[ST_XSLOT] >= 0 ? p[ST_XSLOT] * C * WAVE : 0;
    o[QS_YSO] = p[ST_YSLOT] >= 0 ? p[ST_YSLOT] * C * WAVE : 0;
    o[QS_XDO] = p[ST_XDPOS] >= 0 ? p[ST_XDPOS] * WAVE : 0;
    o[QS_VDO] = p[ST_VDPOS] >= 0 ? p[ST_VDPOS] * WAVE : 0;
    o[QS_MXG] = p[ST_MX] >= 0 ? p[ST_MX] * 16 : 0;
    o[QS_MYG] = p[ST_MY] >= 0 ? p[ST_MY] * 16 : 0;
    o[QS_MVG] = p[ST_MV] >= 0 ? p[ST_MV] * 16 : 0;
  }
  return q;
}

size_t quad_lds_bytes(int S, int C, int nmat, int R, int ndeep) {
  return (size_t)C * nmat * R * 4 * 8 + 64 * 8 + (size_t)C * QCOLS * 8 + (size_t)C * ndeep * WAVE * 8 +
         ((size_t)S * (QCOLS / 2) + 15) / 16 * 16;
}

constexpr int QMW_INTS = 20;
enum {
  QM_XT = 0, QM_YT, QM_MXB, QM_MYB, QM_MVB, QM_VSO, QM_FL, QM_XSO, QM_YSO,
  QM_XS,
  QM_YS,
  QM_VOUT,
  QM_MXG, QM_MYG, QM_MVG,
  QM_NXSO,
  QM_SID,
  QM_XID,
  QM_YID,
  QM_NYSO
};
PHY_HD inline int qmw_tag(int trip, int ph, int id) { return ((trip * 2 + ph) << 13) | id; }
constexpr int QMW_MAXSTEPS = 8192;
constexpr int QM_XW = 32;
constexpr int QM_YW = 64;
constexpr int QM_RW = 128;
// ... 156 lines not shown
  unsigned long long extra = 0;
  std::vector<int> vec_of;
  std::vector<int> prog;
  std::vector<int> mat_branch, gpos;
  std::vector<uint8_t> tips;
  std::vector<double> w;
  std::vector<int32_t> peel;
};

int make_problem(int S, int P, int C, int rooted, int kind, const uint8_t* tipcodes, const double* weights,
                 const int32_t* peel, int max_draws, Problem& pb) {
  if (S < 3) return fail(PHY_EINVAL, "need S >= 3 taxa");
  if (P < 1) return fail(PHY_EINVAL, "need P >= 1 patterns");
  if (C < 1 || C > 16) return fail(PHY_EINVAL, "C must be in 1..16");
  if (kind < PHY_JC69 || kind > PHY_GTR) return fail(PHY_EINVAL, "unknown model");
  if (max_draws < 1) return fail(PHY_EINVAL, "max_draws must be >= 1");
  if (!tipcodes || !weights || !peel) return fail(PHY_EINVAL, "NULL input array");
  for (size_t k = 0; k < (size_t)S * P; ++k)
    if (tipcodes[k] > 15) return fail(PHY_EINVAL, "tip code > 15");
  pb = Problem();
  pb.S = S; pb.P = P; pb.C = C; pb.rooted = rooted ? 1 : 0; pb.kind = kind; pb.max_draws = max_draws;
  pb.B = rooted ? 2 * S - 2 : 2 * S - 3;
  pb.Ppad = nblk_for(P, 2) * 2 * WAVE;
  int rc = build_program(S, peel, pb.rooted, pb.prog, pb.mat_branch, pb.nslots, pb.ndeep);
  if (rc) return rc;
  pb.nsteps = S - 1; pb.nmat = (int)pb.mat_branch.size();
  if (S > 16000 || pb.ndeep > 127)
    return fail(PHY_EINVAL, "tree too large for the packed program (S <= 16000, deep stack <= 127)");
  pb.vec_of.assign(16, -1);
  {
    bool present[16] = {false};
    for (size_t k = 0; k < (size_t)S * P; ++k) present[tipcodes[k]] = true;
    present[15] = true;
    for (int j = 0; j < 4; ++j) pb.vec_of[1 << j] = j;
    int R = 4;
    for (int t = 0; t < 16; ++t)
      if (present[t] && pb.vec_of[t] < 0) {
        pb.extra |= (unsigned long long)t << (4 * (R - 4));
        pb.vec_of[t] = R++;
      }
    pb.R = R;
  }
  if (((size_t)C * pb.B + 16 + 1024) * sizeof(double) > LDS_CAP)
    return fail(PHY_EINVAL, "too many branches x categories for the finalize's LDS (C * B must be <= 19,440)");
  if (lds_bytes(S, C, pb.R, 3, 1, 0) > LDS_CAP) return fail(PHY_EINVAL, "too many taxa for one block's tips in LDS");
  if (pb.nmat != pb.B) return fail(PHY_EINVAL, "internal: one matrix per branch expected");
  pb.gpos.assign(pb.B, -1);
  for (int m = 0; m < pb.nmat; ++m) pb.gpos[pb.mat_branch[m]] = m;
  for (int b = 0; b < pb.B; ++b)
    if (pb.gpos[b] < 0) return fail(PHY_EINVAL, "internal: branch " + std::to_string(b) + " not in the program");
  pb.tips.assign(tipcodes, tipcodes + (size_t)S * P);
  pb.w.assign(weights, weights + P);
  pb.peel.assign(peel, peel + 3 * (S - 1));
  return PHY_OK;
}

std::vector<uint8_t> pack_tips(const Problem& pb, const CladePlan* cp = nullptr) {
  const int S = pb.S, P = pb.P, row = (pb.Ppad + (cp ? CC_COLS : 0)) / 2;
  const uint8_t pad = (uint8_t)pb.vec_of[15];
  std::vector<uint8_t> tips((size_t)S * row, (uint8_t)(pad | (pad << 4)));
  auto setnib = [&](int t, int i, int code) {
    const uint8_t v = (uint8_t)pb.vec_of[code];
    uint8_t& b = tips[(size_t)t * row + i / 2];
    b = (i & 1) ? (uint8_t)((b & 0x0F) | (v << 4)) : (uint8_t)((b & 0xF0) | v);
  };
  for (int t = 0; t < S; ++t) {
    for (int i = 0; i < P; ++i) setnib(t, i, pb.tips[(size_t)t * P + i]);
    const int ci = cp ? cp->clade_of_tip[t] : -1;
    if (ci < 0) continue;
    for (int j = 0; j < cp->ncls[ci]; ++j)
      setnib(t, pb.Ppad + j, pb.tips[(size_t)t * P + cp->rep[(size_t)ci * CC_COLS + j]]);
  }
  return tips;
}

struct Prefs {
  int wg_budget = 0, cols = 0, lds_budget = 0;
  int deep = 0;
  bool recompute = true;
  bool fin = true;
  bool qfuse = true;
  bool quad = true, qmw = true;
  int cc_mode = -1;
  int engine = 0;
  bool rescale = false;
};

Prefs prefs_from_env() {
  auto num = [](const char* name, int dflt, int lo, int hi) {
    const char* v = getenv(name);
    return v ? std::max(lo, std::min(hi, atoi(v))) : dflt;
  };
  auto flag = [](const char* name) {
    const char* v = getenv(name);
    return v ? atoi(v) != 0 : true;
  };
  Prefs p;
  p.lds_budget = num("PHY_LDS_BUDGET", 0, 16384, INT_MAX);
  p.wg_budget = num("PHY_WG_BUDGET", 0, 1, INT_MAX);
  p.cols = num("PHY_COLS", 0, 0, 2);
  p.deep = num("PHY_DEEP", 0, 0, 2);
  p.recompute = flag("PHY_RECOMPUTE");
  p.fin = flag("PHY_FIN");
  p.qfuse = flag("PHY_QFUSE");
  p.quad = flag("PHY_QUAD");
  p.qmw = flag("PHY_QMW");
  p.cc_mode = num("PHY_CLADE_COMPRESSION", -1, -1, 1);
  p.engine = num("PHY_ENGINE", 0, 0, 3);
  return p;
}

inline long wg_cap_for(const Problem& pb, int wg_budget, int cu_count) {
  return std::min<long>((long)nblk_for(pb.P, 1) * pb.max_draws,
                        (long)std::max(wg_budget, 4 * cu_count) + pb.max_draws);
}

struct SweepPlan {
  int cu_count = 256;
  int K = 1;
  bool lat = false;
  int nblk = 0;
  int cap_m = 0, nchunks = 0;
  int ndl = 0;
  bool deep_lds = false;
  int nrec = 0;
  int wg_resident = 512;
  size_t lds = 0;
  long wg_need = 0;
  std::vector<int> prog, records;
  int engine = 0;
  bool quad_ok = false, qmw_ok = false;
  bool cc_ok = false;
  int cc_nchunks = 0, cc_nrec = 0;
};

int plan_lds(const Problem& pb, const Prefs& prefs, int cu_count, SweepPlan& plan) {
  int K = prefs.cols;
  bool lat = false;
  if (!K) {
    K = pb.C <= 8 ? 2 : 1;
    if (K == 2 && (long)pb.max_draws * nblk_for(pb.P, 1) * pb.C <= 4L * cu_count) {
      K = 1;
      lat = true;
    }
  }
  if (K == 2 && pb.C > 8) return fail(PHY_EINVAL, "two columns per lane need C <= 8");
  if ((size_t)std::max(pb.nslots, pb.ndeep) * K * 2 * pb.C * WAVE * 16 >= (size_t)OOB)
    return fail(PHY_EINVAL, "per-workgroup scratch region too large for 32-bit buffer offsets");
  const int nb = nblk_for(pb.P, K);
  int ndl = 0;
  auto cap_for = [&](size_t budget) {
    int cap = pb.nmat;
    while (cap > 3 && lds_bytes(pb.S, pb.C, pb.R, cap, K, ndl) > budget) --cap;
    return cap;
  };
  auto fits = [&](int cap, size_t budget) {
    return lds_bytes(pb.S, pb.C, pb.R, cap, K, ndl) <= budget && cap >= std::min(pb.nmat, MIN_CAP);
  };
  const int by_waves = std::max(1, 4 * waves_per_simd(K, lat) / pb.C);
  int cap = 0;
  auto place = [&](size_t budget, bool last) -> bool {
    if (prefs.deep != 2) {
      ndl = pb.ndeep;
      cap = cap_for(budget);
      if (fits(cap, budget) || (prefs.deep == 1 && last)) return true;
      if (prefs.deep == 1) return false;
    }
    for (ndl = pb.ndeep - 1; ndl >= 0; --ndl) {
      if (prefs.deep == 2) ndl = 0;
      cap = cap_for(budget);
      if (fits(cap, budget)) return true;
    }
    ndl = 0;
    cap = cap_for(budget);
    return false;
  };
  if (prefs.lds_budget > 0) {
    place(std::min<size_t>(LDS_CAP, (size_t)prefs.lds_budget), true);
  } else {
    for (int t = by_waves; t >= 1; --t)
      if (place(LDS_CAP / t, t == 1)) break;
  }
  const size_t lds = lds_bytes(pb.S, pb.C, pb.R, cap, K, ndl);
  if (lds > LDS_CAP) return fail(PHY_EINVAL, "tree too large for LDS (tips of one block)");
  std::vector<int> prog = pb.prog;
  int nch = 0, nrec = 0;
  const int rc = assign_chunks(prog, pb.nsteps, pb.nmat, cap, prefs.recompute, nch, nrec);
  if (rc) return rc;
  plan.cu_count = cu_count; plan.K = K; plan.lat = lat; plan.nblk = nb;
  plan.wg_resident = cu_count * std::min<int>(by_waves, (int)(LDS_CAP / lds));
  const long budget = prefs.wg_budget > 0 ? prefs.wg_budget : plan.wg_resident;
  plan.wg_need = std::min<long>((long)pb.max_draws * nb, budget + pb.max_draws);
  plan.records = K == 2 ? batched_records(prog, K, pb.C, pb.R) : pack_program(prog);
  plan.prog = std::move(prog);
  plan.cap_m = cap; plan.nchunks = nch; plan.nrec = nrec; plan.ndl = ndl; plan.lds = lds;
  plan.deep_lds = ndl > 0 && ndl == pb.ndeep;
  return PHY_OK;
}

int select_clades(const Problem& pb, int mode, CladePlan& cp) {
  cp = CladePlan();
  if (mode == 0 || pb.C > 8) return PHY_OK;
  PeelTree t;
  int rc = parse_peel(pb.S, pb.peel.data(), pb.rooted, t);
  if (rc || (rc = plan_clades(t, pb.P, pb.tips.data(), mode, cp))) return rc;
  if (cp.ncl > 0 && (cp.nmat != pb.nmat || cp.nblk * CC_COLS != pb.Ppad ||
                     (size_t)clade_nslots(cp, pb.S) * 2 * 2 * pb.C * WAVE * 16 >= (size_t)OOB))
    cp = CladePlan();
  return PHY_OK;
}

int plan_clade_records(const Problem& pb, const Prefs& prefs, const CladePlan& cp, SweepPlan& plan,
                       std::vector<int>& recs) {
  plan.cc_ok = false;
  if (cp.ncl == 0 || plan.K != 2) return PHY_OK;
  if (cp.ndeep > pb.ndeep) return PHY_OK;
  std::vector<int> raw;
  int rc = clade_records(cp, pb.S, pb.C, pb.R, plan.cap_m, prefs.recompute, raw, recs, plan.cc_nchunks, plan.cc_nrec);
  if (rc) return rc;
  plan.cc_ok = true;
  return PHY_OK;
}

struct QuadPlan {
  size_t lds = 0, mw_lds = 0;
  std::vector<int> prog;
  QmwPlan mw;
};

QuadPlan plan_quad(const Problem& pb, SweepPlan& plan) {
  QuadPlan q;
  q.lds = quad_lds_bytes(pb.S, pb.C, pb.nmat, pb.R, pb.ndeep);
  plan.quad_ok = q.lds + EIG_LEN * sizeof(double) <= LDS_CAP;
  plan.qmw_ok = false;
  if (!plan.quad_ok) return q;
  q.prog = quad_program(plan.prog, pb.nsteps, pb.C, pb.R);
  for (int W = std::min(QMW_MAXW, 16 / pb.C); W >= 2 && !plan.qmw_ok; --W) {
    if (!quad_mw_plan(plan.prog, q.prog, pb.nsteps, W, q.mw)) continue;
    q.mw_lds = qmw_lds_bytes(pb.S, pb.C, pb.nmat, pb.R, q.mw.nslot);
    plan.qmw_ok = q.mw_lds + EIG_LEN * sizeof(double) <= LDS_CAP;
  }
  return q;
}

inline int qfin_bper(const Problem& pb) { return std::max(1, std::min((pb.B + 15) / 16, QFIN_ITEMS / pb.C)); }
inline int qfin_nspl(const Problem& pb) { return (pb.B + qfin_bper(pb) - 1) / qfin_bper(pb); }

enum LaunchPath {
  PATH_CLASS = 0,
  PATH_QUAD,
  PATH_QUAD_MW,
  PATH_PATTERN_CC,
  PATH_PATTERN,
};
struct LaunchChoice {
  int path = PATH_PATTERN;
  int gx = 1;
  int g_direct = 0;
  int fin = 0;
  int qf = 0;
  int gsum_in = 0;
  int fin_qf = 0;
  bool qfin = false;
  bool quad_build = false;
  bool quad() const { return path == PATH_QUAD || path == PATH_QUAD_MW; }
  bool cc() const { return path == PATH_PATTERN_CC; }
  const double* eig = nullptr;
  const int *mat_branch = nullptr, *gpos = nullptr;
};

LaunchChoice choose_launch(const Problem& pb, const Prefs& prefs, const SweepPlan& plan, int n, bool eig_given) {
  LaunchChoice ch;
  const int C = pb.C, B = pb.B;
  if (plan.engine == 1) {
    ch.path = PATH_CLASS;
    return ch;
  }
  if (plan.quad_ok && prefs.quad && prefs.cols == 0 && n <= QUAD_MAX_DRAWS && !prefs.rescale) {
    ch.path = (plan.qmw_ok && prefs.qmw) ? PATH_QUAD_MW : PATH_QUAD;
    ch.quad_build = eig_given;
    const int nb = (pb.P + QCOLS - 1) / QCOLS;
    ch.gx = std::max(1, std::min(nb, (4 * plan.cu_count) / (C * n)));
    ch.gsum_in = ch.gx <= 16 ? 1 : 0;
    ch.fin_qf = prefs.qfuse ? 1 : 0;
    ch.qfin = ch.gx <= QFIN_SLOTS && C * qfin_bper(pb) <= QFIN_ITEMS && 8 * C <= 128 && prefs.qfuse;
  } else {
    const int budget = prefs.wg_budget > 0 ? prefs.wg_budget : plan.wg_resident;
    ch.gx = std::max(1, std::min(plan.nblk, (budget + n - 1) / n));
    ch.g_direct = ch.gx == 1 ? 1 : 0;
    const bool cc = plan.cc_ok && prefs.cc_mode != 0 && plan.K == 2 && !prefs.rescale && ch.gx == 1;
    ch.path = cc ? PATH_PATTERN_CC : PATH_PATTERN;
    const size_t room = plan.lds - tip_nib_bytes(pb.S, plan.K) - 16 * 4 * sizeof(double);
    ch.fin = (ch.g_direct && prefs.fin && ((size_t)C * B + 8 * C) * 8 <= room) ? 1 : 0;
    ch.qf = (ch.fin && prefs.qfuse && ((size_t)C * B + 8 * C + QG_SHARED) * 8 <= room) ? 1 : 0;
    ch.gsum_in = (!ch.g_direct && ch.gx <= 16) ? 1 : 0;
    ch.fin_qf = (!ch.fin && prefs.qfuse) ? 1 : 0;
  }
  if (!ch.qfin && ((size_t)C * B + 16 + 1024 + QG_SHARED) * sizeof(double) > LDS_CAP) ch.fin_qf = 0;
  return ch;
}

}

#endif
```

### phylostan_amd/engine.py

```python
import ctypes

import numpy as np

from . import _lib
from . import models


class EvalResult:

    __slots__ = ("loglik", "grad_blens", "grad_rs", "grad_ps", "grad_freq_root", "grad_rates", "grad_freqs",
                 "dLdP", "site_ll")

    def __init__(self, vec, B, C, site_ll=None):
        o = 1 + B + 2 * C
        og = o + 4 + 10
        self.loglik = float(vec[0])
        self.grad_blens = vec[1:1 + B].copy()
        self.grad_rs = vec[1 + B:1 + B + C].copy()
        self.grad_ps = vec[1 + B + C:o].copy()
        self.grad_freq_root = vec[o:o + 4].copy()
        self.grad_rates = vec[o + 4:o + 10].copy()
        self.grad_freqs = vec[o + 10:og].copy()
        self.dLdP = vec[og:og + C * B * 16].reshape(C, B, 4, 4).copy() if len(vec) >= og + C * B * 16 else None
        self.site_ll = site_ll

    def as_dict(self):
        return {k: getattr(self, k) for k in self.__slots__}


def _ptr(a):
    return a.ctypes.data_as(ctypes.c_void_p)


def plan_records(peel0, rooted, C, R, cols, cap, recompute=True):
    peel = np.ascontiguousarray(peel0, dtype=np.int32)
    S = peel.shape[0] + 1
    program = np.zeros((S - 1, 16), dtype=np.int32)
    records = np.zeros((S - 1, 16), dtype=np.int32)
    nmat, nch = ctypes.c_int(), ctypes.c_int()
    _lib.check(_lib.load().phy_plan_records(S, _ptr(peel), int(bool(rooted)), int(C), int(R), int(cols), int(cap),
                                            int(bool(recompute)), _ptr(program), _ptr(records),
                                            ctypes.byref(nmat), ctypes.byref(nch)), "phy_plan_records")
    return program, records, nmat.value, nch.value


CLADE_FACTS = ("clades", "l_steps", "u_steps", "l_matrices", "u_matrices", "rounds", "class_columns", "blocks",
               "scratch_entries", "depth", "n_chunks", "recomputed")
CLADE_FIELDS = ("node", "internal_nodes", "classes", "maxmult", "first_step", "last_step")
CLADE_MAX = 8
CLADE_MODES = {"off": 0, "on": 1, "auto": -1}


def _clade_dict(facts, clades):
    out = dict(zip(CLADE_FACTS, (int(v) for v in facts)))
    out["clade_list"] = [dict(zip(CLADE_FIELDS, (int(v) for v in clades[k]))) for k in range(out["clades"])]
    return out


def clade_plan(tipcodes, peel0, rooted, C, R, cap, recompute=True, mode=-1):
    tip = np.ascontiguousarray(tipcodes, dtype=np.uint8)
    peel = np.ascontiguousarray(peel0, dtype=np.int32)
    S, P = tip.shape
    nblk = (P + 127) // 128
    facts = np.zeros(12, dtype=np.int32)
    clades = np.zeros((CLADE_MAX, 6), dtype=np.int32)
    program = np.zeros((S - 1, 16), dtype=np.int32)
    records = np.zeros((S - 1, 16), dtype=np.int32)
    mat_branch = np.zeros(2 * S - 2, dtype=np.int32)
    cls_of = np.full((CLADE_MAX, nblk * 128), -1, dtype=np.int32)
    members = np.full((CLADE_MAX * ((P + 3) // 4 * 4), 128), -1, dtype=np.int32)
    rep = np.full((CLADE_MAX, 128), -1, dtype=np.int32)
    _lib.check(_lib.load().phy_clade_plan(S, P, int(C), int(bool(rooted)), _ptr(tip), _ptr(peel), int(R), int(cap),
                                          int(bool(recompute)), int(mode), _ptr(facts), _ptr(clades), _ptr(program),
                                          _ptr(records), _ptr(mat_branch), _ptr(cls_of), _ptr(members), _ptr(rep)),
               "phy_clade_plan")
    out = _clade_dict(facts, clades)
    if out["clades"]:
        n, r = out["clades"], out["rounds"]
        out.update(program=program, records=records, mat_branch=mat_branch[:out["l_matrices"] + out["u_matrices"]],
                   cls_of=cls_of[:n], members=members[:n * r].reshape(n, r, 128), rep=rep[:n])
    return out


PLAN_FACTS = ("nsteps", "nslots", "depth", "R", "cols", "latency_plan", "nblocks", "matrices_per_chunk", "n_chunks",
              "deep_lds_entries", "recomputed", "resident_workgroups", "lds_bytes", "quad_ok", "quad_waves",
              "quad_span", "quad_slots")
LAUNCH_FACTS = ("path", "gx", "g_direct", "fin", "qf", "gsum_in", "quad_build")
LAUNCH_PATHS = ("class", "quad", "quad_mw", "pattern_cc", "pattern")


def plan_sweep(tipcodes, peel0, rooted, C, max_draws, cu_count, n_draws, wg_budget=0, cols=0, lds_budget=0, deep=0,
               recompute=True, clade_mode=-1, rescaling=False):
    tip = np.ascontiguousarray(tipcodes, dtype=np.uint8)
    peel = np.ascontiguousarray(peel0, dtype=np.int32)
    S, P = tip.shape
    facts = np.zeros(36, dtype=np.int32)
    _lib.check(_lib.load().phy_plan_sweep(S, P, int(C), int(bool(rooted)), _ptr(tip), _ptr(peel), int(max_draws),
                                          int(cu_count), int(wg_budget), int(cols), int(lds_budget), int(deep),
                                          int(bool(recompute)), int(clade_mode), int(bool(rescaling)), int(n_draws),
                                          _ptr(facts)), "phy_plan_sweep")
    out = dict(zip(PLAN_FACTS, (int(v) for v in facts[:17])))
    out["clade"] = dict(zip(CLADE_FACTS, (int(v) for v in facts[17:29])))
    out["launch"] = dict(zip(LAUNCH_FACTS, (int(v) for v in facts[29:36])))
    out["launch"]["path"] = LAUNCH_PATHS[out["launch"]["path"]]
    return out


class TreeLikelihood:

    _pending = 0

    def __init__(self, tipcodes, weights, peel0, rooted, model, C, max_draws=1, device=0, devices=None,
                 rescaling=False):
        self.lib = _lib.load()
        tipcodes = np.ascontiguousarray(tipcodes, dtype=np.uint8)
        self.S, self.P = tipcodes.shape
        self.C = int(C)
        self.rooted = bool(rooted)
        self.model = models.MODEL_IDS[model] if isinstance(model, str) else int(model)
        self.max_draws = int(max_draws)
        w = np.ascontiguousarray(weights, dtype=np.float64)
        peel = np.ascontiguousarray(peel0, dtype=np.int32)
        if w.shape != (self.P,):
            raise ValueError("weights must have shape (P,)")
        if peel.shape != (self.S - 1, 3):
            raise ValueError("peel must have shape (S-1, 3)")
        ctx = ctypes.c_void_p()
        if devices is not None:
            devs = np.ascontiguousarray(devices, dtype=np.int32)
            _lib.check(self.lib.phy_create_multi(self.S, self.P, self.C, int(self.rooted), self.model,
                                                 _ptr(tipcodes), _ptr(w), _ptr(peel), self.max_draws,
                                                 int(devs.size), _ptr(devs), ctypes.byref(ctx)), "phy_create_multi")
        else:
            _lib.check(self.lib.phy_create(self.S, self.P, self.C, int(self.rooted), self.model,
                                           _ptr(tipcodes), _ptr(w), _ptr(peel), self.max_draws,
                                           int(device), ctypes.byref(ctx)), "phy_create")
        self.ctx = ctx
        self.B = self.lib.phy_num_branches(ctx)
        self.outlen = self.lib.phy_output_len(ctx)
        self.model_len = 10 + 2 * self.C
        if rescaling:
            self.set_rescaling(True)

    @classmethod
    def from_data(cls, data, model, C, **kw):
        return cls(data.tipcodes, data.weights, data.peel0, data.rooted, model, C, **kw)

    def close(self):
        if getattr(self, "ctx", None):
            self.lib.phy_destroy(self.ctx)
            self.ctx = None

    def __del__(self):
        try:
            self.close()
        except Exception:
            pass

    def program_info(self):
        vals = [ctypes.c_int() for _ in range(4)]
        _lib.check(self.lib.phy_program_info(self.ctx, *[ctypes.byref(v) for v in vals]),
                   "phy_program_info")
        out = dict(zip(("nsteps", "nslots", "depth", "nblocks"), [v.value for v in vals]))
# ... 224 lines not shown
```

Baseline: 1.538 million evals/s.

## Pack clade gather/scatter tables into LDS tip rows instead of global table

Clade-compression index tables (class column, plane position, prefix/count, header) are now packed as extra byte/short rows appended to the tip buffer. They are staged into LDS along with the tips, so the CC kernel path computes gather and scatter offsets from LDS instead of issuing global loads followed by vmcnt waits. LDS sizing for the clade path is recomputed, with the matrix cap per chunk shrunk to fit. This adds LDS pressure that may reduce matrices per chunk or occupancy. It also adds a diagnostic API and a PHY_CLADE_NODES env filter.

```diff
diff --git a/include/phylo_hip_diag.h b/include/phylo_hip_diag.h
--- a/include/phylo_hip_diag.h
+++ b/include/phylo_hip_diag.h
@@ -18,6 +18,11 @@
 int phy_clade_plan(int S, int P, int C, int rooted, const uint8_t* tipcodes, const int32_t* peel, int R, int cap,
                    int recompute, int mode, int* facts, int* clades, int32_t* program, int32_t* records,
                    int32_t* mat_branch, int32_t* cls_of, int32_t* members, int32_t* rep);
+
+#define PHY_ROWS_FACTS 12
+int phy_clade_rows(int S, int P, int C, int rooted, const uint8_t* tipcodes, const int32_t* peel, int max_draws,
+                   int cu_count, int cols, int lds_budget, int deep, int recompute, int clade_mode, int* facts,
+                   uint8_t* rows, int32_t* table, int32_t* program);
 
 #define PHY_PLAN_QUAD 13
 #define PHY_PLAN_CLADE 17
diff --git a/phylostan_amd/_lib.py b/phylostan_amd/_lib.py
--- a/phylostan_amd/_lib.py
+++ b/phylostan_amd/_lib.py
@@ -31,6 +31,8 @@
                                         ctypes.c_void_p, _c_int_p, _c_int_p]),
     "phy_clade_plan": (ctypes.c_int, [ctypes.c_int] * 4 + [ctypes.c_void_p, ctypes.c_void_p] + [ctypes.c_int] * 4 +
                        [ctypes.c_void_p] * 8),
+    "phy_clade_rows": (ctypes.c_int, [ctypes.c_int] * 4 + [ctypes.c_void_p, ctypes.c_void_p] + [ctypes.c_int] * 7 +
+                       [ctypes.c_void_p] * 4),
     "phy_plan_sweep": (ctypes.c_int, [ctypes.c_int] * 4 + [ctypes.c_void_p, ctypes.c_void_p] + [ctypes.c_int] * 10 +
                        [ctypes.c_void_p]),
     "phy_set_clade_compression": (ctypes.c_int, [ctypes.c_void_p, ctypes.c_int]),
diff --git a/phylostan_amd/csrc/phylo_hip.hip b/phylostan_amd/csrc/phylo_hip.hip
--- a/phylostan_amd/csrc/phylo_hip.hip
+++ b/phylostan_amd/csrc/phylo_hip.hip
@@ -185,15 +185,12 @@
   long long grows_stride;
   int qfused, kind;
   int* escr;
-  union {
-    const int* cc;
-    const int* tree_of_row;
-  };
+  const int* tree_of_row;
   union {
     int cc_ncl;
     int fo_stride;
   };
-  int cc_nL, cc_ncol, cc_spos, cc_pre, cc_cnt;
+  int cc_nL, cc_ncol;
 };
 
 __device__ __forceinline__ __amdgpu_buffer_rsrc_t make_rsrc(const void* base, uint32_t bytes) {
@@ -556,7 +553,7 @@
 __device__ unsigned long long g_tt[TT_DRAWS * 16][TT_EV];
 #define TT_MARK(i)                                                                   \
   do {                                                                               \
-    if (draw >= TT_DRAW0 && draw < TT_DRAW0 + TT_DRAWS && lane == 0)                 \
+    if ((i) < TT_EV && draw >= TT_DRAW0 && draw < TT_DRAW0 + TT_DRAWS && lane == 0)  \
       g_tt[(draw - TT_DRAW0) * 16 + wv][(i)] = __builtin_amdgcn_s_memtime();         \
   } while (0)
 #else
@@ -585,9 +582,11 @@
   const int ncolwg = C * WAVE;
 
   unsigned char* tipl = lds_raw;
-  double* tvec = reinterpret_cast<double*>(lds_raw + tip_nib_bytes(a.S, K));
-  double* mats0 = tvec + 64;
-  if (threadIdx.x < 64) {
+  const int trows = CC ? a.S + CC_XROWS * a.cc_ncl : a.S;
+  double* tvec = reinterpret_cast<double*>(lds_raw + tip_nib_bytes(trows, K));
+  const int tvn = CC ? a.R * 4 : 64;
+  double* mats0 = tvec + tvn;
+  if (threadIdx.x < tvn) {
     const unsigned b = threadIdx.x >> 2, j = threadIdx.x & 3;
     const unsigned m = b < 4 ? (1u << b) : (unsigned)(a.extra >> (4 * (b - 4))) & 15u;
     tvec[threadIdx.x] = (double)((m >> j) & 1u);
@@ -718,6 +717,16 @@
   const uint32_t cw = (uint32_t)c * (WAVE * 16);
   const uint32_t plane_half = (uint32_t)a.nblk * (estr / 2);
   const uint32_t cwp = (uint32_t)c * (uint32_t)a.nblk * (WAVE * K * 16);
+  const unsigned char* const xrow = tipl + (size_t)a.S * (WAVE * K / 2);
+  constexpr int XCL = CC_XROWS * (WAVE * K / 2);
+  auto cls_col = [&](int cl, int k) __attribute__((always_inline)) -> uint32_t {
+    const unsigned j = xrow[cl * XCL + k * WAVE + lane];
+    return j == (unsigned)CC_NOCLS ? OOB : (((j >> 6) * 2u * (unsigned)ncolwg + (j & 63u)) << 4) + cw;
+  };
+  auto pos_off = [&](int cl, int k) __attribute__((always_inline)) -> uint32_t {
+    const unsigned v = *reinterpret_cast<const unsigned short*>(xrow + cl * XCL + CC_COLS + (k * WAVE + lane) * 2);
+    return v == (unsigned)CC_NOPOS ? OOB : v * 16u + cwp;
+  };
   for (int trip = 0; trip < trips; ++trip) {
     const bool passLF = CC && trip == 0, passLR = CC && trip == trips - 1;
     const int blk = CC ? ((passLF || passLR) ? a.nblk : trip - 1) : vg + trip * VG;
@@ -740,7 +749,7 @@
       uint32_t* dst = reinterpret_cast<uint32_t*>(tipl);
       const int rowq = a.Ppad / 8;
       constexpr int wq = WAVE * K / 8;
-      const int nq = a.S * wq;
+      const int nq = trows * wq;
       const int nthr = C * WAVE, t0 = c * WAVE + lane;
       for (int k0 = t0; k0 < nq; k0 += nthr * 8) {
         uint32_t buf[8];
@@ -763,14 +772,10 @@
     V4 top[K], proot[K];
 #pragma unroll
     for (int k = 0; k < K; ++k) top[k] = proot[k] = {0.0, 0.0, 0.0, 0.0};
-    #define GATHER(ch, so, out) do {                                                         \
-      const int* gt_ = a.cc + CC_HDR + ((-2 - (ch)) * a.nblk + blk) * (WAVE * K) + lane;     \
-      uint32_t gc_[K];                                                                       \
-      _Pragma("unroll")                                                                      \
-      for (int k = 0; k < K; ++k) gc_[k] = (uint32_t)gt_[k * WAVE] + cw;                     \
-      _Pragma("unroll")                                                                      \
-      for (int k = 0; k < K; ++k) out[k] = ld_v4(srd_scr, gc_[k] + (so), half_bytes);        \
-      WAIT_VMCNT0();                                                                         \
+    #define GATHER(ch, so, out) do {                                                                \
+      _Pragma("unroll")                                                                             \
+      for (int k = 0; k < K; ++k) out[k] = ld_v4(srd_scr, cls_col(-2 - (ch), k) + (so), half_bytes);  \
+      WAIT_VMCNT0();                                                                                \
     } while (0)
     #define FSTEP(s, dcur, dnext, st, sn) do {                                            \
       {                                                                                   \
@@ -949,16 +954,12 @@
       for (int k = 0; k < K; ++k) cx_[k] = cy_[k] = lofs[k];                     \
       if constexpr (CC) {   \
         if (ok && r.st.x < -1) {                                                 \
-          const int* gt_ = a.cc + CC_HDR + ((-2 - r.st.x) * a.nblk + blk) * (WAVE * K) + lane;  \
       _Pragma("unroll")                                                          \
-          for (int k = 0; k < K; ++k) cx_[k] = (uint32_t)gt_[k * WAVE] + cw;     \
-          WAIT_VMCNT0();                                                         \
+          for (int k = 0; k < K; ++k) cx_[k] = cls_col(-2 - r.st.x, k);          \
         }                                                                        \
         if (ok && r.st.y < -1) {                                                 \
-          const int* gt_ = a.cc + CC_HDR + ((-2 - r.st.y) * a.nblk + blk) * (WAVE * K) + lane;  \
       _Pragma("unroll")                                                          \
-          for (int k = 0; k < K; ++k) cy_[k] = (uint32_t)gt_[k * WAVE] + cw;     \
-          WAIT_VMCNT0();                                                         \
+          for (int k = 0; k < K; ++k) cy_[k] = cls_col(-2 - r.st.y, k);          \
         }                                                                        \
       }                                                                          \
       _Pragma("unroll")                                                          \
@@ -1005,14 +1006,9 @@
         CHAIN_UP(vst, acc_, out);                                                         \
       }                                                                                   \
     } while (0)
-    #define PLANE_PUT(ch, po, r) do {                                                    \
-      const int* sp_ = a.cc + a.cc_spos + ((-2 - (ch)) * a.nblk + blk) * (WAVE * K) + lane;  \
-      uint32_t so_[K];                                                                   \
-      _Pragma("unroll")                                                                  \
-      for (int k = 0; k < K; ++k) so_[k] = (uint32_t)sp_[k * WAVE] + cwp + (uint32_t)(po);  \
-      WAIT_VMCNT0();                                                                     \
-      _Pragma("unroll")                                                                  \
-      for (int k = 0; k < K; ++k) st_v4(srd_scr, so_[k], plane_half, r[k]);              \
+    #define PLANE_PUT(ch, po, r) do {                                                                       \
+      _Pragma("unroll")                                                                                     \
+      for (int k = 0; k < K; ++k) st_v4(srd_scr, pos_off(-2 - (ch), k) + (uint32_t)(po), plane_half, r[k]);  \
     } while (0)
     #define RSTEP_V(s, cs, cn, XT, YT) do {                                               \
       const Step& st = cs.st;                                                     \
@@ -1130,15 +1126,18 @@
       int rlo = CC ? a.cc_nL : 0, rhi = nsteps - 1;
       if constexpr (CC) {
         if (passLR) {
-          rlo = a.cc[4 * sg];
-          rhi = a.cc[4 * sg + 1];
-          const int mm = a.cc[4 * sg + 3];
+          const int* hd = reinterpret_cast<const int*>(xrow + sg * XCL);
+          const unsigned short* run0 = reinterpret_cast<const unsigned short*>(xrow + sg * XCL + CC_COLS);
+          rlo = __builtin_amdgcn_readfirstlane(hd[0]);
+          rhi = __builtin_amdgcn_readfirstlane(hd[1]);
+          const int mm = __builtin_amdgcn_readfirstlane(hd[2]);
           uint32_t pre[K], cnt[K];
 #pragma unroll
           for (int k = 0; k < K; ++k) {
-            pre[k] = (uint32_t)a.cc[a.cc_pre + sg * (WAVE * K) + k * WAVE + lane] + cwp +
-                     (uint32_t)(nsteps + sg * a.nblk) * estr;
-            cnt[k] = (uint32_t)a.cc[a.cc_cnt + sg * (WAVE * K) + k * WAVE + lane];
+            const int j = k * WAVE + lane;
+            const uint32_t p0 = run0[j], pn = run0[j + 1 < CC_COLS ? j + 1 : j];
+            pre[k] = p0 * 16u + cwp + (uint32_t)(nsteps + sg * a.nblk) * estr;
+            cnt[k] = (j + 1 < CC_COLS ? pn : (uint32_t)hd[3]) - p0;
           }
 #pragma unroll
           for (int k = 0; k < K; ++k) topr[k] = {0.0, 0.0, 0.0, 0.0};
@@ -2025,7 +2024,7 @@
 struct CladeBuffers {
   uint8_t* tips = nullptr;
   double* w = nullptr;
-  int *prog = nullptr, *tab = nullptr;
+  int* prog = nullptr;
   int *matbr = nullptr, *gpos = nullptr;
 };
 }
@@ -2079,7 +2078,7 @@
                   c->d_eig,   c->d_inner, c->d_model,   c->d_blens,   c->d_out,        c->d_site,
                   c->d_scratch, c->d_dstk, c->d_gslot,  c->d_sslot, c->d_grows, c->d_in, c->d_qprog, c->d_qscr,
                   c->d_qfpart, c->d_qfcnt, c->d_mprog, c->d_escr,
-                  c->ccd.tips, c->ccd.w, c->ccd.prog, c->ccd.tab, c->ccd.matbr, c->ccd.gpos};
+                  c->ccd.tips, c->ccd.w, c->ccd.prog, c->ccd.matbr, c->ccd.gpos};
   for (void* p : ptrs)
     if (p) (void)hipFree(p);
   if (c->h_in) (void)hipHostFree(c->h_in);
@@ -2147,27 +2146,28 @@
 
 int build_clade_plan(phy_ctx* c) {
   CladeBuffers& d = c->ccd;
-  void* old[] = {d.tips, d.w, d.prog, d.tab, d.matbr, d.gpos};
+  void* old[] = {d.tips, d.w, d.prog, d.matbr, d.gpos};
   for (void* p : old)
     if (p) (void)hipFree(p);
   d = CladeBuffers();
   c->plan.cc_ok = false;
   const Problem& pb = c->pb;
-  int rc = select_clades(pb, c->prefs.cc_mode, c->cc);
+  int rc = select_clades(pb, c->prefs.cc_mode, c->cc, &c->prefs.cc_only);
   if (rc) return rc;
   const CladePlan& cp = c->cc;
   if (cp.ncl == 0) return PHY_OK;
-  const std::vector<uint8_t> tips = pack_tips(pb, &cp);
+  std::vector<uint8_t> tips = pack_tips(pb, &cp);
+  const std::vector<uint8_t> rows = clade_rows(cp);
+  tips.insert(tips.end(), rows.begin(), rows.end());
   std::vector<double> w(pb.Ppad + CC_COLS, 0.0);
   std::copy(pb.w.begin(), pb.w.end(), w.begin());
   std::vector<int> gpos(pb.B, -1);
   for (int m = 0; m < cp.nmat; ++m) gpos[cp.mat_branch[m]] = m;
-  const std::vector<int> tab = clade_table(cp, pb.S, pb.C);
   if ((rc = dalloc(&d.tips, tips.size())) || (rc = dalloc(&d.w, w.size())) ||
-      (rc = dalloc(&d.prog, (size_t)(pb.S - 1) * USTEP)) || (rc = dalloc(&d.tab, tab.size())) ||
+      (rc = dalloc(&d.prog, (size_t)(pb.S - 1) * USTEP)) ||
       (rc = dalloc(&d.matbr, (size_t)cp.nmat)) || (rc = dalloc(&d.gpos, gpos.size())))
     return rc;
-  if ((rc = upload(d.tips, tips)) || (rc = upload(d.w, w)) || (rc = upload(d.tab, tab)) ||
+  if ((rc = upload(d.tips, tips)) || (rc = upload(d.w, w)) ||
       (rc = upload(d.matbr, cp.mat_branch)))
     return rc;
   return upload(d.gpos, gpos);
@@ -2265,10 +2265,8 @@
   if (ch.cc()) {
     const CladePlan& cp = ctx->cc;
     a.tips = ctx->ccd.tips; a.weights = ctx->ccd.w; a.Ppad = pb.Ppad + CC_COLS; a.nslots = clade_nslots(cp, pb.S);
-    a.cc = ctx->ccd.tab; a.cc_ncl = cp.ncl; a.cc_nL = cp.nL; a.cc_ncol = cp.maxcls;
-    a.cc_spos = CC_HDR + cp.ncl * cp.nblk * CC_COLS;
-    a.cc_pre = a.cc_spos + cp.ncl * cp.nblk * CC_COLS;
-    a.cc_cnt = a.cc_pre + cp.ncl * CC_COLS;
+    a.cap_m = pl.cc_cap_m;
+    a.cc_ncl = cp.ncl; a.cc_nL = cp.nL; a.cc_ncol = cp.maxcls;
   }
   return a;
 }
@@ -2517,7 +2515,7 @@
     const int* prog = ch.cc() ? ctx->ccd.prog : ctx->d_prog;
     void* kargs[] = {(void*)&sa, (void*)&prog};
     HIP_TRY(hipLaunchKernel(sweep_kernel_for(pl.K, pl.lat, pl.deep_lds, ctx->prefs.rescale, ch.cc()), dim3(gx, n),
-                            dim3(C * WAVE), kargs, pl.lds, st));
+                            dim3(C * WAVE), kargs, ch.cc() ? pl.cc_lds : pl.lds, st));
   }
   HIP_TRY(hipGetLastError());
   if (ctx->timing) HIP_TRY(hipEventRecord(e1, st));
@@ -2867,7 +2865,7 @@
   if ((rc = plan_lds(pb, prefs, cu_count, plan))) return rc;
   CladePlan cp;
   std::vector<int> recs;
-  if ((rc = select_clades(pb, prefs.cc_mode, cp)) || (rc = plan_clade_records(pb, prefs, cp, plan, recs))) return rc;
+  if ((rc = select_clades(pb, prefs.cc_mode, cp, &prefs.cc_only)) || (rc = plan_clade_records(pb, prefs, cp, plan, recs))) return rc;
   const QuadPlan quad = plan_quad(pb, plan);
   const LaunchChoice ch = choose_launch(pb, prefs, plan, n_draws, n_draws <= EIG_HOST_MAX);
   const int head[PHY_PLAN_QUAD] = {pb.nsteps, pb.nslots, pb.ndeep, pb.R, plan.K, plan.lat ? 1 : 0, plan.nblk,
@@ -2879,6 +2877,35 @@
   const int tail[PHY_PLAN_FACTS - PHY_PLAN_LAUNCH] = {ch.path, ch.gx, ch.g_direct, ch.fin, ch.qf, ch.gsum_in,
                                                       ch.quad_build ? 1 : 0};
   std::copy(tail, tail + PHY_PLAN_FACTS - PHY_PLAN_LAUNCH, facts + PHY_PLAN_LAUNCH);
+  return PHY_OK;
+}
+
+int phy_clade_rows(int S, int P, int C, int rooted, const uint8_t* tipcodes, const int32_t* peel, int max_draws,
+                   int cu_count, int cols, int lds_budget, int deep, int recompute, int clade_mode, int* facts,
+                   uint8_t* rows, int32_t* table, int32_t* program) {
+  if (!facts || cu_count < 1 || cols < 0 || cols > 2 || deep < 0 || deep > 2 || clade_mode < -1 || clade_mode > 1)
+    return fail(PHY_EINVAL, "phy_clade_rows: bad argument");
+  const std::vector<double> w((size_t)std::max(P, 1), 1.0);
+  Problem pb;
+  int rc = make_problem(S, P, C, rooted, PHY_JC69, tipcodes, w.data(), peel, max_draws, pb);
+  if (rc) return rc;
+  Prefs prefs = prefs_from_env();
+  if (lds_budget > 0) prefs.lds_budget = std::max(16384, std::min(lds_budget, (int)LDS_CAP));
+  prefs.cols = cols; prefs.deep = deep; prefs.recompute = recompute != 0; prefs.cc_mode = clade_mode;
+  SweepPlan plan;
+  if ((rc = plan_lds(pb, prefs, cu_count, plan))) return rc;
+  CladePlan cp;
+  std::vector<int> recs, raw;
+  if ((rc = select_clades(pb, prefs.cc_mode, cp, &prefs.cc_only)) || (rc = plan_clade_records(pb, prefs, cp, plan, recs, &raw))) return rc;
+  const std::vector<uint8_t> packed = cp.ncl ? clade_rows(cp) : std::vector<uint8_t>();
+  const std::vector<int> tab = cp.ncl ? clade_table(cp, S, C) : std::vector<int>();
+  const int fv[PHY_ROWS_FACTS] = {cp.ncl, cp.nblk, CC_XROWS * cp.ncl, cp.ncl ? (cp.nblk + 1) * (CC_COLS / 2) : 0,
+                                  (int)tab.size(), plan.cap_m, (int)plan.lds, (int)lds_share(prefs, plan),
+                                  plan.cc_cap_m, (int)plan.cc_lds, plan.cc_ok ? 1 : 0, plan.cc_nchunks};
+  std::copy(fv, fv + PHY_ROWS_FACTS, facts);
+  if (rows) std::copy(packed.begin(), packed.end(), rows);
+  if (table) std::copy(tab.begin(), tab.end(), table);
+  if (program && plan.cc_ok) std::copy(raw.begin(), raw.end(), program);
   return PHY_OK;
 }
 
diff --git a/phylostan_amd/csrc/sweep_plan.h b/phylostan_amd/csrc/sweep_plan.h
--- a/phylostan_amd/csrc/sweep_plan.h
+++ b/phylostan_amd/csrc/sweep_plan.h
@@ -54,6 +54,9 @@
 constexpr int CC_MININT = 3;
 constexpr int CC_ROUNDS_U = 8;
 constexpr int CC_HDR = 4 * CC_MAXCL;
+constexpr int CC_XROWS = 6;
+constexpr int CC_NOCLS = 0xFF;
+constexpr int CC_NOPOS = 0xFFFF;
 
 constexpr int PSTEP = 8;
 enum {
@@ -416,7 +419,8 @@
 constexpr long CC_CLADE_CYCLES = 7000;
 constexpr long CC_FIXED_CYCLES = 6000;
 
-int plan_clades(const PeelTree& t, int P, const uint8_t* tipcodes, int mode, CladePlan& cp) {
+int plan_clades(const PeelTree& t, int P, const uint8_t* tipcodes, int mode, CladePlan& cp,
+                const std::vector<int>* only_in = nullptr) {
   const int S = t.S, N = 2 * S - 1;
   cp = CladePlan();
   cp.nblk = (P + CC_COLS - 1) / CC_COLS;
@@ -477,13 +481,16 @@
     for (int p = 0; p < P; ++p) ++sz[cid[v][p]];
     return *std::max_element(sz.begin(), sz.end());
   };
+  static const std::vector<int> every;
+  const std::vector<int>& only = (mode == 1 && only_in) ? *only_in : every;
   long gain = 0;
   std::vector<int> walk{t.root};
   while (!walk.empty()) {
     const int v = walk.back();
     walk.pop_back();
     if (v < S) continue;
-    bool take = v != t.root && count[v] > 0 && nint[v] >= CC_MININT && cp.ncl < CC_MAXCL;
+    bool take = v != t.root && count[v] > 0 && nint[v] >= CC_MININT && cp.ncl < CC_MAXCL &&
+                (only.empty() || std::find(only.begin(), only.end(), v) != only.end());
     int mm = 0;
     if (take) {
       mm = mult_of(v);
@@ -602,6 +609,37 @@
   }
   (void)S;
   return tab;
+}
+
+std::vector<uint8_t> clade_rows(const CladePlan& cp) {
+  constexpr int RB = CC_COLS / 2;
+  const int row = (cp.nblk + 1) * RB, pcols = cp.nblk * CC_COLS;
+  std::vector<uint8_t> rows((size_t)CC_XROWS * cp.ncl * row, 0xFF);
+  auto at = [&](int ci, int b, int o) -> uint8_t& {
+    return rows[(size_t)(CC_XROWS * ci + o / RB) * row + (size_t)b * RB + o % RB];
+  };
+  auto put16 = [&](int ci, int b, int q, int v) {
+    at(ci, b, CC_COLS + 2 * q) = (uint8_t)(v & 0xFF);
+    at(ci, b, CC_COLS + 2 * q + 1) = (uint8_t)(v >> 8);
+  };
+  for (int ci = 0; ci < cp.ncl; ++ci) {
+    for (int p = 0; p < pcols; ++p) {
+      const int j = cp.cls_of[(size_t)ci * pcols + p];
+      if (j >= 0) at(ci, p / CC_COLS, p % CC_COLS) = (uint8_t)j;
+    }
+    int run = 0;
+    for (int j = 0; j < CC_COLS; ++j) {
+      put16(ci, cp.nblk, j, run);
+      for (int r = 0; r < cp.rounds; ++r) {
+        const int p = cp.members[((size_t)ci * cp.rounds + r) * CC_COLS + j];
+        if (p < 0) break;
+        put16(ci, p / CC_COLS, p % CC_COLS, run++);
+      }
+    }
+    const int hdr[4] = {cp.lo[ci], cp.hi[ci], cp.maxmult[ci], run};
+    for (int k = 0; k < 16; ++k) at(ci, cp.nblk, k) = (uint8_t)((unsigned)hdr[k / 4] >> (8 * (k % 4)));
+  }
+  return rows;
 }
 
 void clade_facts(const CladePlan& cp, int S, int nchunks, int nrec, bool on, int* facts, int* clades) {
@@ -924,6 +962,7 @@
   bool qfuse = true;
   bool quad = true, qmw = true;
   int cc_mode = -1;
+  std::vector<int> cc_only;
   int engine = 0;
   bool rescale = false;
 };
@@ -948,6 +987,14 @@
   p.quad = flag("PHY_QUAD");
   p.qmw = flag("PHY_QMW");
   p.cc_mode = num("PHY_CLADE_COMPRESSION", -1, -1, 1);
+  if (const char* e = getenv("PHY_CLADE_NODES"))
+    for (const char* q = e; *q;) {
+      char* end = nullptr;
+      const long n = strtol(q, &end, 10);
+      if (end == q) break;
+      p.cc_only.push_back((int)n);
+      q = *end == ',' ? end + 1 : end;
+    }
   p.engine = num("PHY_ENGINE", 0, 0, 3);
   return p;
 }
@@ -974,6 +1021,9 @@
   bool quad_ok = false, qmw_ok = false;
   bool cc_ok = false;
   int cc_nchunks = 0, cc_nrec = 0;
+  int cc_rows = 0;
+  int cc_cap_m = 0;
+  size_t cc_lds = 0;
 };
 
 int plan_lds(const Problem& pb, const Prefs& prefs, int cu_count, SweepPlan& plan) {
@@ -1040,26 +1090,50 @@
   return PHY_OK;
 }
 
-int select_clades(const Problem& pb, int mode, CladePlan& cp) {
+int select_clades(const Problem& pb, int mode, CladePlan& cp, const std::vector<int>* only = nullptr) {
   cp = CladePlan();
   if (mode == 0 || pb.C > 8) return PHY_OK;
   PeelTree t;
   int rc = parse_peel(pb.S, pb.peel.data(), pb.rooted, t);
-  if (rc || (rc = plan_clades(t, pb.P, pb.tips.data(), mode, cp))) return rc;
+  if (rc || (rc = plan_clades(t, pb.P, pb.tips.data(), mode, cp, only))) return rc;
   if (cp.ncl > 0 && (cp.nmat != pb.nmat || cp.nblk * CC_COLS != pb.Ppad ||
+                     cp.nblk * CC_COLS >= CC_NOPOS ||
                      (size_t)clade_nslots(cp, pb.S) * 2 * 2 * pb.C * WAVE * 16 >= (size_t)OOB))
     cp = CladePlan();
   return PHY_OK;
 }
 
+inline size_t lds_share(const Prefs& prefs, const SweepPlan& plan) {
+  const size_t step = LDS_CAP / std::max<size_t>(1, LDS_CAP / std::max<size_t>(1, plan.lds));
+  if (prefs.lds_budget > 0) return std::min<size_t>(step, (size_t)prefs.lds_budget);
+  return LDS_CAP / (size_t)std::max(1, plan.wg_resident / std::max(1, plan.cu_count));
+}
+PHY_HD inline size_t clade_lds_bytes(int S, int rows, int C, int R, int cap_m, int ndl) {
+  return tip_nib_bytes(S + rows, 2) + (size_t)R * 4 * sizeof(double) + (size_t)C * cap_m * R * 32 +
+         (size_t)C * tail_doubles(2, ndl) * 8;
+}
+inline int clade_cap(const Problem& pb, const CladePlan& cp, const SweepPlan& plan, size_t share) {
+  int cap = plan.cap_m;
+  while (cap >= 3 && clade_lds_bytes(pb.S, CC_XROWS * cp.ncl, pb.C, pb.R, cap, plan.ndl) > share) --cap;
+  return cap;
+}
+
 int plan_clade_records(const Problem& pb, const Prefs& prefs, const CladePlan& cp, SweepPlan& plan,
-                       std::vector<int>& recs) {
+                       std::vector<int>& recs, std::vector<int>* raw_out = nullptr) {
   plan.cc_ok = false;
+  plan.cc_rows = plan.cc_cap_m = plan.cc_nchunks = plan.cc_nrec = 0;
+  plan.cc_lds = 0;
   if (cp.ncl == 0 || plan.K != 2) return PHY_OK;
   if (cp.ndeep > pb.ndeep) return PHY_OK;
+  const int cap = clade_cap(pb, cp, plan, lds_share(prefs, plan));
+  if (cap < 3 || cap < std::min(pb.nmat, MIN_CAP)) return PHY_OK;
   std::vector<int> raw;
-  int rc = clade_records(cp, pb.S, pb.C, pb.R, plan.cap_m, prefs.recompute, raw, recs, plan.cc_nchunks, plan.cc_nrec);
+  int rc = clade_records(cp, pb.S, pb.C, pb.R, cap, prefs.recompute, raw, recs, plan.cc_nchunks, plan.cc_nrec);
   if (rc) return rc;
+  if (raw_out) *raw_out = std::move(raw);
+  plan.cc_rows = CC_XROWS * cp.ncl;
+  plan.cc_cap_m = cap;
+  plan.cc_lds = clade_lds_bytes(pb.S, plan.cc_rows, pb.C, pb.R, cap, plan.ndl);
   plan.cc_ok = true;
   return PHY_OK;
 }
@@ -1132,7 +1206,8 @@
     ch.g_direct = ch.gx == 1 ? 1 : 0;
     const bool cc = plan.cc_ok && prefs.cc_mode != 0 && plan.K == 2 && !prefs.rescale && ch.gx == 1;
     ch.path = cc ? PATH_PATTERN_CC : PATH_PATTERN;
-    const size_t room = plan.lds - tip_nib_bytes(pb.S, plan.K) - 16 * 4 * sizeof(double);
+    const size_t room = cc ? plan.cc_lds - tip_nib_bytes(pb.S + plan.cc_rows, plan.K) - pb.R * 4 * sizeof(double)
+                           : plan.lds - tip_nib_bytes(pb.S, plan.K) - 16 * 4 * sizeof(double);
     ch.fin = (ch.g_direct && prefs.fin && ((size_t)C * B + 8 * C) * 8 <= room) ? 1 : 0;
     ch.qf = (ch.fin && prefs.qfuse && ((size_t)C * B + 8 * C + QG_SHARED) * 8 <= room) ? 1 : 0;
     ch.gsum_in = (!ch.g_direct && ch.gx <= 16) ? 1 : 0;
diff --git a/phylostan_amd/engine.py b/phylostan_amd/engine.py
--- a/phylostan_amd/engine.py
+++ b/phylostan_amd/engine.py
@@ -79,6 +79,35 @@
         n, r = out["clades"], out["rounds"]
         out.update(program=program, records=records, mat_branch=mat_branch[:out["l_matrices"] + out["u_matrices"]],
                    cls_of=cls_of[:n], members=members[:n * r].reshape(n, r, 128), rep=rep[:n])
+    return out
+
+
+ROWS_FACTS = ("clades", "blocks", "boundary_rows", "row_bytes", "table_ints", "matrices_per_chunk", "lds_bytes",
+              "lds_share", "cc_matrices_per_chunk", "cc_lds_bytes", "cc_ok", "cc_n_chunks")
+
+
+def clade_rows(tipcodes, peel0, rooted, C, max_draws, cu_count, cols=0, lds_budget=0, deep=0, recompute=True,
+               clade_mode=-1):
+    tip = np.ascontiguousarray(tipcodes, dtype=np.uint8)
+    peel = np.ascontiguousarray(peel0, dtype=np.int32)
+    S, P = tip.shape
+    nblk = (P + 127) // 128
+    facts = np.zeros(len(ROWS_FACTS), dtype=np.int32)
+    rows = np.zeros(CLADE_MAX * 6 * (nblk + 1) * 64, dtype=np.uint8)
+    table = np.zeros(4 * CLADE_MAX + 2 * CLADE_MAX * (nblk + 1) * 128, dtype=np.int32)
+    program = np.zeros((S - 1, 16), dtype=np.int32)
+    _lib.check(_lib.load().phy_clade_rows(S, P, int(C), int(bool(rooted)), _ptr(tip), _ptr(peel), int(max_draws),
+                                          int(cu_count), int(cols), int(lds_budget), int(deep), int(bool(recompute)),
+                                          int(clade_mode), _ptr(facts), _ptr(rows), _ptr(table), _ptr(program)),
+               "phy_clade_rows")
+    out = dict(zip(ROWS_FACTS, (int(v) for v in facts)))
+    n = out["clades"]
+    if n:
+        pc, h = nblk * 128, 4 * CLADE_MAX
+        out.update(rows=rows[:n * 6 * (nblk + 1) * 64].reshape(n, 6, nblk + 1, 64), header=table[:4 * n].reshape(n, 4),
+                   cls=table[h:h + n * pc].reshape(n, pc), spos=table[h + n * pc:h + 2 * n * pc].reshape(n, pc),
+                   pre=table[h + 2 * n * pc:h + 2 * n * pc + n * 128].reshape(n, 128),
+                   cnt=table[h + 2 * n * pc + n * 128:h + 2 * n * pc + 2 * n * 128].reshape(n, 128), program=program)
     return out
 
 
```

Result: faster. 1.571 million evals/s (median of 6 runs) (+2.2%).
